# seang123/Masters-Thesis

Hardware: AMD Instinct MI355X
Metric: caption-tokens/sec training (20k-voxel enc, 512 LSTM, B=64) (higher is better)
Workload: dtype f32; 1 GPU; config 2: AttemptFour NIC.py dense 20000->512 encoder + BatchNorm + 512-unit LSTM, V=5001, T=15, B=64/GPU; global_batch=64, seq_len=15, parallelism=dp1, replay=launch plan

## Files before the change

### include/tnt_hip.h

```cpp
#ifndef TNT_HIP_H
#define TNT_HIP_H
#include <stdint.h>

#ifdef __cplusplus
extern "C" {
#endif

#define TNT_ACT_NONE 0
#define TNT_ACT_LEAKY 1
#define TNT_ACT_RELU 2
#define TNT_ACT_TANH 3

int32_t tnt_version(void);

int32_t tnt_gemm_f32(const float* A, const float* B, float* C, const float* bias, float* pre,
                     int32_t M, int32_t N, int32_t K, int32_t lda, int32_t ldb, int32_t ldc,
                     int32_t transA, int32_t transB, int32_t act, float slope,
                     int32_t accumulate, int32_t splitk, float* work, void* stream);
int32_t tnt_gemm_blas_f32(const float* A, const float* B, float* C, int32_t M, int32_t N, int32_t K,
                          int32_t lda, int32_t ldb, int32_t ldc, int32_t transA, int32_t transB,
                          int32_t accumulate, void* stream);

int32_t tnt_gemm_lt_f32(const float* A, const float* B, float* C, const float* bias, int32_t M, int32_t N, int32_t K,
                        int32_t lda, int32_t ldb, int32_t ldc, int32_t transA, int32_t transB, void* stream);
// ... 46 lines not shown
int32_t tnt_dense_dw_adam_fin_f32(const float* x, const float* dpre, float* theta, float* m, float* v, float l2,
                                  const float* partial, int32_t k0, int32_t k1, const float* sq_override,
                                  const float* lr_t_dev, float beta1, float beta2, float eps, float clipnorm,
                                  const uint32_t* guard, int32_t N, int32_t E, int32_t Bk, int32_t ldx, void* stream);
int32_t tnt_adam_fin_f32(float* theta, float* m, float* v, const float* grad, const int32_t* span_seg,
                         const int64_t* span_off, const int32_t* span_len, const float* sq_override, int32_t nspan, float eps,
                         float clipnorm, const tnt_finalize_desc* fin, const float* met, int32_t nmet, float* ring,
                         int32_t ring_rows, uint32_t* ring_t, void* stream);

int32_t tnt_gemm_f32_tile(const float* A, const float* B, float* C, const float* bias, float* pre,
                          int32_t M, int32_t N, int32_t K, int32_t lda, int32_t ldb, int32_t ldc,
                          int32_t transA, int32_t transB, int32_t act, float slope,
                          int32_t accumulate, int32_t splitk, float* work, int32_t bm, int32_t bn,
                          void* stream);

int32_t tnt_dropout_mask4_u8(uint8_t* out, int64_t n, int32_t nsites, float rate, uint64_t seed, uint32_t site0,
                             uint32_t step, const uint32_t* step_dev, void* stream);
int32_t tnt_dropout_f32(const float* x, float* y, int32_t rows, int32_t cols, int32_t ld,
                        int32_t tmajor_B, int32_t lwidth, int32_t lcol0, int32_t rows_per_site,
                        float rate, uint64_t seed, uint32_t site, uint32_t step,
                        const uint32_t* step_dev, void* stream);
int32_t tnt_dropout_metric_f32(const float* x, float* y, int32_t rows, int32_t cols, int32_t ld, int32_t tmajor_B,
                               int32_t lwidth, int32_t lcol0, int32_t rows_per_site, float rate, uint64_t seed,
                               uint32_t site, uint32_t step, const uint32_t* step_dev, const float* alpha,
                               float* partial, int32_t T, int32_t B, int32_t R, void* stream);
int32_t tnt_dropout2_f32(const float* x, float* y, int32_t rows, int32_t cols, int32_t ld, int32_t tmajor_B_a,
                         int32_t lwidth_a, int32_t lcol0_a, int32_t rows_per_site_a, float rate_a, uint32_t site_a,
                         int32_t tmajor_B_b, int32_t lwidth_b, int32_t lcol0_b, int32_t rows_per_site_b, float rate_b,
                         uint32_t site_b, uint64_t seed, uint32_t step, const uint32_t* step_dev, void* stream);

int32_t tnt_act_bwd_f32(const float* pre, const float* dy, float* dx, int64_t n, int32_t act,
                        float slope, void* stream);
int32_t tnt_bias_act_drop_bwd_f32(const float* dy, const float* pre, float* dx, float* dbias, int32_t rows, int32_t cols,
                                  int32_t ld, int32_t act, float slope, int32_t tmajor_B, int32_t lwidth, int32_t lcol0,
                                  float rate, uint64_t seed, uint32_t site, const uint32_t* step_dev, const float* x1,
                                  float* out1, int32_t rows1, int32_t C1, int32_t ld1, void* stream);

int32_t tnt_bn_nchunk(int32_t rows);
int32_t tnt_batchnorm_fwd_f32(const float* x, const float* gamma, const float* beta,
                              float* mov_mean, float* mov_var, float* y, float* xhat,
                              float* inv_std, int32_t rows, int32_t C, int32_t ldy,
                              int32_t training, float eps, float momentum, float* work,
                              void* stream);
int32_t tnt_batchnorm_fwd_drop_f32(const float* x, const float* gamma, const float* beta,
                                   float* mov_mean, float* mov_var, float* y, float* xhat,
                                   float* inv_std, int32_t rows, int32_t C, int32_t ldy,
                                   int32_t training, float eps, float momentum, float* work,
                                   float rate, uint64_t seed, uint32_t site, const uint32_t* step_dev,
                                   void* stream);
int32_t tnt_batchnorm_bwd_f32(const float* dy, const float* xhat, const float* gamma,
                              const float* inv_std, float* dx, float* dgamma, float* dbeta,
                              int32_t rows, int32_t C, int32_t lddy, int32_t training,
                              float* work, void* stream);
int32_t tnt_batchnorm_bwd_act_f32(const float* dy, const float* xhat, const float* gamma,
                              const float* inv_std, float* dx, float* dgamma, float* dbeta,
                              int32_t rows, int32_t C, int32_t lddy, int32_t training,
                              float* work, const float* act_pre, float slope, void* stream);

int32_t tnt_batchnorm_stats_f32(const float* x, int32_t rows, int32_t C, float* part, void* stream);
int32_t tnt_batchnorm_apply_stats_f32(const float* part_all, int32_t nrep, const float* x, const float* gamma,
                                      const float* beta, float* mov_mean, float* mov_var, float* y, float* xhat,
                                      float* inv_std, int32_t rows, int32_t C, int32_t ldy, float eps, float momentum,
                                      float* mean_work, void* stream);
int32_t tnt_batchnorm_dx_f32(const float* dy, int32_t lddy, const float* xhat, const float* gamma, const float* inv_std,
                             const float* dgamma_sum, const float* dbeta_sum, float* dx, int32_t rows, int32_t C,
                             int32_t n_total, void* stream);

int32_t tnt_locally_dense_fwd_split_f32(const float* x, int32_t ldx, const int32_t* idx, const int32_t* vgoff,
                                        const int32_t* vreg, const int32_t* rfirst, int32_t NV,
                                        const float* W, const float* bias, float* pre, float* y,
                                        float* partial, int32_t B, int32_t R, int32_t D, float slope,
                                        int32_t x_voxel_major, void* stream);
int32_t tnt_locally_dense_bwd_split_f32(const float* x, int32_t ldx, const int32_t* idx, const int32_t* vgoff,
                                        const int32_t* vreg, const int32_t* vfirst, int32_t NV,
                                        const float* dpre, float* dW, float* db, int32_t B, int32_t R,
                                        int32_t D, int32_t x_voxel_major, void* stream);

int32_t tnt_dense_fwd_stream_f32(const float* x, const float* w, float* part, int32_t B, int32_t E, int32_t K,
                                 int32_t ldx, int32_t ldw, int32_t nsplit, void* stream);

int32_t tnt_dense_fwd_stream_gram_f32(const float* x, const float* w, float* part, float* gx_part, float* w2_part,
                                      int32_t B, int32_t E, int32_t K, int32_t ldx, int32_t ldw, int32_t nsplit,
                                      void* stream);
int32_t tnt_dense_gram_norm_f32(const float* dpre, const float* pre, const float* bias, const float* gx_part,
                                int32_t nsplit, const float* w2_part, int32_t nw2, float l2, float* partial,
                                int32_t nslot, int32_t Bk, int32_t E, void* stream);
int32_t tnt_dense_gram_norm_spans_f32(const float* dpre, const float* pre, const float* bias, const float* gx_part,
                                      int32_t nsplit, const float* w2_part, int32_t nw2, float l2, float* partial,
                                      int32_t nslot, int32_t Bk, int32_t E, const float* theta, const float* grad,
                                      const int32_t* span_seg, const int64_t* span_off, const int32_t* span_len,
                                      const float* seg_l2, float* span_partial, int32_t nspan, void* stream);

int32_t tnt_dense_dw_skinny_f32(const float* x, const float* dpre, float* dw, int32_t N, int32_t E,
                                int32_t Bk, int32_t ldx, void* stream);

int32_t tnt_dense_dw_sqnorm_f32(const float* x, const float* dpre, const float* theta, float l2, float* partial,
                                int32_t nslot, int32_t N, int32_t E, int32_t Bk, int32_t ldx, void* stream);
int32_t tnt_dense_dw_adam_f32(const float* x, const float* dpre, float* theta, float* m, float* v, float l2,
                              const float* sq, const float* sq_override, const float* lr_t_dev, float beta1,
                              float beta2, float eps, float clipnorm, const uint32_t* guard, int32_t N, int32_t E,
                              int32_t Bk, int32_t ldx, void* stream);

int32_t tnt_enc_tail_fwd_f32(const float* y, const float* gamma, const float* beta, float* mov_mean,
                             float* mov_var, float* out, float* xhat, float* inv_std, int32_t rows,
                             int32_t C, int32_t ldo, int32_t training, float eps, float momentum,
                             float r_feat, float r_lstm, uint64_t seed, uint32_t site_feat,
                             uint32_t site_lstm, const uint32_t* step_dev, void* stream);
int32_t tnt_enc_tail_fwd_sk_f32(const float* part, int32_t nsplit, const float* bias, float* pre, float slope,
                                const float* gamma, const float* beta, float* mov_mean, float* mov_var, float* out,
                                float* xhat, float* inv_std, int32_t rows, int32_t C, int32_t ldo, int32_t training,
                                float eps, float momentum, float r_feat, float r_lstm, uint64_t seed,
                                uint32_t site_feat, uint32_t site_lstm, const uint32_t* step_dev, void* stream);
int32_t tnt_enc_tail_fwd_sk_emb_f32(const float* part, int32_t nsplit, const float* bias, float* pre, float slope,
                                    const float* gamma, const float* beta, float* mov_mean, float* mov_var, float* out,
                                    float* xhat, float* inv_std, int32_t rows, int32_t C, int32_t ldo, int32_t training,
                                    float eps, float momentum, float r_feat, float r_lstm, uint64_t seed,
                                    uint32_t site_feat, uint32_t site_lstm, const uint32_t* step_dev,
                                    const float* emb_table, const int32_t* emb_ids, float* emb_out, int32_t emb_B,
                                    int32_t emb_T, int32_t emb_V, float emb_rate, uint32_t emb_site, void* stream);
int32_t tnt_enc_tail_bwd_f32(const float* dout, const float* xhat, const float* gamma, const float* inv_std,
                             const float* pre, float* dpre, float* dgamma, float* dbeta, float* dbias,
                             int32_t rows, int32_t C, int32_t ldo, float r_feat, float r_lstm, float slope,
                             uint64_t seed, uint32_t site_feat, uint32_t site_lstm,
                             const uint32_t* step_dev, void* stream);
int32_t tnt_enc_tail_bwd_drop_f32(const float* dout, const float* xhat, const float* gamma, const float* inv_std,
                                  const float* pre, float* dpre, float* dgamma, float* dbeta, float* dbias, int32_t rows,
                                  int32_t C, int32_t ldo, float r_feat, float r_lstm, float slope, uint64_t seed,
                                  uint32_t site_feat, uint32_t site_lstm, const uint32_t* step_dev, float* drop_x,
                                  int32_t drop_rows, int32_t drop_cols, int32_t drop_ld, int32_t drop_tmajor_B,
                                  int32_t drop_lwidth, int32_t drop_lcol0, float drop_rate, uint32_t drop_site,
                                  void* stream);

int32_t tnt_layernorm_fwd_f32(const float* x, const float* gamma, const float* beta, float* y,
                              float* xhat, float* inv_std, int32_t rows, int32_t C,
                              int32_t ldy, float eps, void* stream);
int32_t tnt_layernorm_bwd_f32(const float* dy, const float* xhat, const float* gamma,
                              const float* inv_std, float* dx, float* dgamma, float* dbeta,
                              int32_t rows, int32_t C, int32_t lddy, float* work, void* stream);

int32_t tnt_colsum_f32(const float* x, float* out, int32_t rows, int32_t C, int32_t ld,
                       float* work, void* stream);
int32_t tnt_colsum4_f32(const float* x0, float* out0, int32_t rows0, int32_t C0, int32_t ld0, const float* x1, float* out1,
                        int32_t rows1, int32_t C1, int32_t ld1, const float* x2, float* out2, int32_t rows2, int32_t C2,
                        int32_t ld2, const float* x3, float* out3, int32_t rows3, int32_t C3, int32_t ld3, void* stream);
int32_t tnt_colsum2_f32(const float* x0, float* out0, int32_t rows0, int32_t C0, int32_t ld0, const float* x1,
                        float* out1, int32_t rows1, int32_t C1, int32_t ld1, void* stream);

int32_t tnt_embedding_fwd_f32(const float* table, const int32_t* ids, float* out, int32_t B,
                              int32_t T, int32_t E, int32_t ldo, int32_t V, void* stream);
int32_t tnt_embedding_fwd_drop_f32(const float* table, const int32_t* ids, float* out, float* out_drop,
                                   int32_t B, int32_t T, int32_t E, int32_t ldo, int32_t V, float rate,
                                   uint64_t seed, uint32_t site, uint32_t step, const uint32_t* step_dev,
                                   void* stream);
int32_t tnt_embedding_fwd_drop2_f32(const float* table, const int32_t* ids, float* out, float* out_drop,
                                    int32_t B, int32_t T, int32_t E, int32_t ldo, int32_t V, float rate,
                                    uint64_t seed, uint32_t site, uint32_t step, const uint32_t* step_dev,
                                    float rate2, uint32_t site2, int32_t lwidth2, int32_t lcol0_2, void* stream);
int32_t tnt_embedding_bwd_parts(int32_t B, int32_t T, int32_t E);
int32_t tnt_embedding_bwd_sparse_f32(const float* drows, const int32_t* ids, const int32_t* prev_ids, float* dtable,
                                     float* sq_part, int32_t B, int32_t T, int32_t E, int32_t ldd, int32_t V,
                                     float drop_rate, uint64_t drop_seed, uint32_t drop_site,
                                     const uint32_t* drop_step_dev, int32_t zero_id, void* stream);
int32_t tnt_embedding_bwd_f32(const float* drows, const int32_t* ids, float* dtable,
                              float* sq_norm, float* rowsq_work, int32_t B, int32_t T,
                              int32_t E, int32_t ldd, int32_t V, void* stream);

// ... 260 lines not shown
```

### masters-thesis_amd/_lib.py

```python
import ctypes as C
import os

import torch

_HERE = os.path.dirname(os.path.abspath(__file__))
LIB_PATH = os.environ.get("TNT_HIP_LIB") or os.path.join(_HERE, "csrc", "libtnt_hip.so")

P = C.c_void_p
I32, I64, U32, U64, F32 = C.c_int32, C.c_int64, C.c_uint32, C.c_uint64, C.c_float

SIGNATURES = {
    "tnt_version": [],
    "tnt_gemm_f32": [P, P, P, P, P, I32, I32, I32, I32, I32, I32, I32, I32, I32, F32, I32, I32, P, P],
    "tnt_gemm_fused_f32": [P, P, P, P, P, P, P, I32, I32, I32, I32, I32, I32, I32, I32, I32, P],
    "tnt_gemm_fused_cfg": [I32, I32, I32, I32, I32, I32],
    "tnt_gemm3_f32": [P, P, P, P, P, P, P, I32, I32, I32, I32, I32, I32, I32, I32, I32, I32, P, P, P, I32, P],
    "tnt_gemm3_plan": [I32, I32, I32, I32, I32, I32, I32, P, P],
    "tnt_gemm3_work_floats": [I32, I32, I32, I32, I32],
    "tnt_gemm3_sync_words": [I32, I32, I32, I32],
    "tnt_gemm3_work_arm": [P, I64, P],
    "tnt_gemm3_pair_supported": [I32, I32, I32, I32, I32, I32],
    "tnt_gemm3_pair_f32": [P, P, P],
    "tnt_span_sqnorm_lr_f32": [P, P, P, P, P, P, P, I32, P, P, P, F32, F32, P, P],
    "tnt_dense_gram_norm_spans_lr_f32": [P, P, P, P, I32, P, I32, F32, P, I32, I32, I32, P, P, P, P, P, P, P, I32, P, P, P, F32, F32, P, P],
    "tnt_dense_dw_adam_fin_f32": [P, P, P, P, P, F32, P, I32, I32, P, P, F32, F32, F32, F32, P, I32, I32, I32, I32, P],
    "tnt_adam_fin_f32": [P, P, P, P, P, P, P, P, I32, F32, F32, P, P, I32, P, I32, P, P],
    "tnt_dropout_mask4_u8": [P, I64, I32, F32, U64, U32, U32, P, P],
    "tnt_dropout_f32": [P, P, I32, I32, I32, I32, I32, I32, I32, F32, U64, U32, U32, P, P],
    "tnt_dropout_metric_f32": [P, P, I32, I32, I32, I32, I32, I32, I32, F32, U64, U32, U32, P, P, P, I32, I32, I32, P],
    "tnt_dropout2_f32": [P, P, I32, I32, I32, I32, I32, I32, I32, F32, U32, I32, I32, I32, I32, F32, U32, U64, U32, P, P],
    "tnt_act_bwd_f32": [P, P, P, I64, I32, F32, P],
    "tnt_bn_nchunk": [I32],
    "tnt_batchnorm_fwd_f32": [P, P, P, P, P, P, P, P, I32, I32, I32, I32, F32, F32, P, P],
    "tnt_batchnorm_bwd_f32": [P, P, P, P, P, P, P, I32, I32, I32, I32, P, P],
    "tnt_batchnorm_fwd_drop_f32": [P, P, P, P, P, P, P, P, I32, I32, I32, I32, F32, F32, P, F32, U64, U32, P, P],
    "tnt_batchnorm_bwd_act_f32": [P, P, P, P, P, P, P, I32, I32, I32, I32, P, P, F32, P],
    "tnt_batchnorm_stats_f32": [P, I32, I32, P, P],
    "tnt_batchnorm_apply_stats_f32": [P, I32, P, P, P, P, P, P, P, P, I32, I32, I32, F32, F32, P, P],
    "tnt_batchnorm_dx_f32": [P, I32, P, P, P, P, P, P, I32, I32, I32, P],
    "tnt_layernorm_fwd_f32": [P, P, P, P, P, P, I32, I32, I32, F32, P],
    "tnt_layernorm_bwd_f32": [P, P, P, P, P, P, P, I32, I32, I32, P, P],
    "tnt_colsum_f32": [P, P, I32, I32, I32, P, P],
    "tnt_bias_act_drop_bwd_f32": [P, P, P, P, I32, I32, I32, I32, F32, I32, I32, I32, F32, U64, U32, P, P, P, I32, I32, I32, P],
    "tnt_colsum2_f32": [P, P, I32, I32, I32, P, P, I32, I32, I32, P],
    "tnt_colsum4_f32": [P, P, I32, I32, I32, P, P, I32, I32, I32, P, P, I32, I32, I32, P, P, I32, I32, I32, P],
    "tnt_embedding_fwd_f32": [P, P, P, I32, I32, I32, I32, I32, P],
    "tnt_embedding_bwd_parts": [I32, I32, I32],
    "tnt_attention_front_bwd_parts": [I32, I32, I32],
    "tnt_attention_metric_parts": [I32, I32],
    "tnt_embedding_bwd_sparse_f32": [P, P, P, P, P, I32, I32, I32, I32, I32, F32, U64, U32, P, I32, P],
    "tnt_embedding_bwd_f32": [P, P, P, P, P, I32, I32, I32, I32, I32, P],
    "tnt_lstm_seq_supported": [I32, I32],
    "tnt_lstm_seq_fwd_f32": [P, P, P, P, P, P, I32, I32, P, P, I32, I32, I32, P, P, P, P],
    "tnt_lstm_seq_bwd_work_floats": [I32, I32],
    "tnt_lstm_seq_bwd_f32": [P, P, P, I32, I32, P, P, P, P, I64, I32, I32, I32, P, P, P, P],
    "tnt_lstm_step_fwd_f32": [P, P, P, P, P, P, I32, P, I32, I32, P, P, P, P, P, I32, I32, P, P],
    "tnt_ln_lstm_cell_fwd_f32": [P, P, P, P, P, P, P, P, P, P, P, I32, I32, F32, P],
    "tnt_ln_lstm_cell_bwd_f32": [P, P, P, P, P, P, P, P, P, P, P, P, P, I32, I32, P],
    "tnt_lstm_step_bwd_f32": [P, P, P, P, P, P, P, P, I32, I32, P, P, P, P, P, P, P, I32, I32, P, I32, P, P],
    "tnt_softmax_cce_f32": [P, P, P, P, P, P, I32, I32, I32, F32, I32, I32, P],
    "tnt_softmax_cce_live_f32": [P, P, P, P, P, P, I32, I32, I32, F32, P, P, P],
    "tnt_softmax_cce_smooth_f32": [P, P, P, P, P, P, I32, I32, I32, F32, F32, P],
    "tnt_softmax_cce_unlikely_f32": [P, P, P, P, P, P, I32, I32, I32, I32, F32, F32, P],
    "tnt_onehot_argmax_f32": [P, P, I32, I32, I32, P],
    "tnt_beam_topk_f32": [P, P, P, I32, I32, I32, I32, I32, P, P, P, P, P],
    "tnt_beam_step_f32": [P, I32, P, P, I32, I32, I32, I32, P, P, P, P, P, P, I32, I32, P, P, P],
    "tnt_beam_step_diverse_f32": [P, I32, P, P, I32, I32, I32, I32, P, P, P, P, P, P, I32, I32, P, P, I32, F32, P],
    "tnt_decode_constrain_f32": [P, I32, I32, I32, I32, P, P, I32, P, P, P, F32, I32, I32, I32, P, I32, P],
    "tnt_consensus_mix_f32": [P, I32, I32, I32, I32, P, I32, P, I32, P, P],
    "tnt_consensus_spread_i32": [P, P, P, I32, I32, P, P, P, P],
    "tnt_guidance_mix_f32": [P, I32, I32, I32, F32, F32, P, I32, P, P],
    "tnt_argmax_rows_f32": [P, P, I32, I32, I32, P],
    "tnt_greedy_feedback_f32": [P, I32, I32, P, I32, P, I32, I32, P, I32, I32, P, I32, P, I32, I32, F32, U64, U32, U32, P,
                                I32, I32, P],
    "tnt_scheduled_feedback_f32": [P, I32, I32, P, I32, P, I32, I32, P, I32, I32, P, I32, P, I32, I32, F32, U64, U32, U32, P,
                                   I32, I32, I32, I32, P, P, U32, U32, P],
    "tnt_scheduled_feedback2_f32": [P, I32, I32, P, I32, P, I32, I32, P, I32, I32, P, I32, P, I32, I32, F32, U64, U32, U32, P,
                                    I32, I32, I32, I32, P, P, U32, U32, F32, U32, I32, I32, P],
    "tnt_enc_tail_fwd_f32": [P, P, P, P, P, P, P, P, I32, I32, I32, I32, F32, F32, F32, F32, U64, U32, U32, P, P],
    "tnt_enc_tail_bwd_f32": [P, P, P, P, P, P, P, P, P, I32, I32, I32, F32, F32, F32, U64, U32, U32, P, P],
    "tnt_enc_tail_bwd_drop_f32": [P, P, P, P, P, P, P, P, P, I32, I32, I32, F32, F32, F32, U64, U32, U32, P, P, I32, I32, I32, I32,
                                  I32, I32, F32, U32, P],
    "tnt_embedding_fwd_drop_f32": [P, P, P, P, I32, I32, I32, I32, I32, F32, U64, U32, U32, P, P],
    "tnt_embedding_fwd_drop2_f32": [P, P, P, P, I32, I32, I32, I32, I32, F32, U64, U32, U32, P, F32, U32, I32, I32, P],
    "tnt_dense_dw_skinny_f32": [P, P, P, I32, I32, I32, I32, P],
    "tnt_dense_dw_sqnorm_f32": [P, P, P, F32, P, I32, I32, I32, I32, I32, P],
    "tnt_dense_dw_adam_f32": [P, P, P, P, P, F32, P, P, P, F32, F32, F32, F32, P, I32, I32, I32, I32, P],
    "tnt_dense_fwd_stream_gram_f32": [P, P, P, P, P, I32, I32, I32, I32, I32, I32, P],
    "tnt_dense_gram_norm_f32": [P, P, P, P, I32, P, I32, F32, P, I32, I32, I32, P],
    "tnt_dense_gram_norm_spans_f32": [P, P, P, P, I32, P, I32, F32, P, I32, I32, I32, P, P, P, P, P, P, P, I32, P],
    "tnt_dense_fwd_stream_f32": [P, P, P, I32, I32, I32, I32, I32, I32, P],
    "tnt_enc_tail_fwd_sk_f32": [P, I32, P, P, F32, P, P, P, P, P, P, P, I32, I32, I32, I32, F32, F32, F32, F32, U64, U32,
                                U32, P, P],
    "tnt_enc_tail_fwd_sk_emb_f32": [P, I32, P, P, F32, P, P, P, P, P, P, P, I32, I32, I32, I32, F32, F32, F32, F32, U64, U32,
                                    U32, P, P, P, P, I32, I32, I32, F32, U32, P],
    "tnt_gru_step_fwd_f32": [P, P, P, P, P, P, I32, I32, P],
    "tnt_gru_step_bwd_f32": [P, P, P, P, P, P, P, P, P, I32, I32, P],
    "tnt_lc_seq_fwd_f32": [P, P, P, P, P, P, P, P, P, P, P, I64, P, P, P, P, P, P, P, I32, I32, I32, I32, I32, I32, F32, F32, F32,
                           I32, U64, U32, U32, P, P, P, P, P],
    "tnt_lc_seq_fwd_work_floats": [I32],
    "tnt_lc_seq_bwd_f32": [P, P, P, P, P, P, P, I64, P, P, P, P, P, P, P, P, P, P, P, I32, I32, I32, I32, I32, I32, F32, F32, F32,
                           I32, U64, U32, U32, P, F32, P, P, P],
    "tnt_lc_seq_fwd_drop_f32": [P, P, P, P, P, P, P, P, P, P, P, I64, P, P, P, P, P, P, P, I32, I32, I32, I32, I32, I32, F32, F32,
                                F32, I32, U64, U32, U32, P, P, F32, U32, P, P, P, P],
    "tnt_lc_seq_bwd_drop_f32": [P, P, P, P, P, P, P, I64, P, P, P, P, P, P, P, P, P, P, P, I32, I32, I32, I32, I32, I32, F32, F32,
                                F32, I32, U64, U32, U32, P, F32, F32, U32, P, P, P],
    "tnt_lc_seq_bwd_work_floats": [I32, I32],
    "tnt_attention_front_bwd_f32": [P, P, P, P, P, P, P, P, I32, I32, I32, F32, P],
    "tnt_attention_front_bwd_drop_f32": [P, P, P, P, P, P, P, P, I32, I32, I32, F32, F32, U64, U32, P, P],
    "tnt_gemm_blas_f32": [P, P, P, I32, I32, I32, I32, I32, I32, I32, I32, I32, P],
    "tnt_gemm_lt_f32": [P, P, P, P, I32, I32, I32, I32, I32, I32, I32, I32, P],
    "tnt_locally_dense_fwd_split_f32": [P, I32, P, P, P, P, I32, P, P, P, P, P, I32, I32, I32, F32, I32, P],
    "tnt_locally_dense_bwd_split_f32": [P, I32, P, P, P, P, I32, P, P, P, I32, I32, I32, I32, P],
    "tnt_sum2_f32": [P, P, P, P, I32, F32, P],
    "tnt_stage_batch_f32": [P, P, P, P, P, P, P, P, P, P, I32, I32, I32, I32, I32, P, I32, P],
    "tnt_stage_batch_map_f32": [P, P, P, P, P, P, P, P, P, P, I32, I32, I32, I32, I32, P, I32, P, P, P, P, P, P, P],
    "tnt_stage_batch_h16": [P, P, P, P, P, P, P, P, P, P, I32, I32, I32, I32, I32, P, I32, P],
    "tnt_stage_batch_masks_f32": [P, P, P, P, P, P, P, P, P, P, I32, I32, I32, I32, I32, P, I32, P, I64, I32, F32, U64, U32, P, P],
    "tnt_scst_cce_f32": [P, I32, I32, P, I32, P, P, I32, P, P, P, I32, F32, P],
    "tnt_caption_score_f32": [P, I32, I32, P, I32, I32, I32, I32, P, P, P, P],
    "tnt_sample_rows_f32": [P, P, I32, I32, I32, F32, I32, U64, U32, U32, P, P],
    "tnt_sample_topkp_f32": [P, P, I32, I32, I32, F32, I32, F32, I32, U64, U32, U32, P, P],
    "tnt_sqdiff_mean_f32": [P, P, I64, F32, P],
    "tnt_sum_f32": [P, P, I32, F32, P],
    "tnt_l2_total_f32": [P, P, I32, P, P],
    "tnt_seg_sqnorm_f32": [P, P, P, P, P, P, P, P, P, P, P, I32, I32, P],
    "tnt_span_sqnorm_f32": [P, P, P, P, P, P, P, I32, P],
    "tnt_step_finalize_f32": [P, P, P, P, P, P, I32, P, P, P, P, I32, F32, P, P, I32, P, P, I32, P, P, I32, F32, P, P, P, P,
                              F32, F32, P, P],
    "tnt_adam_f32": [P, P, P, P, P, P, P, P, P, P, I32, F32, P, F32, F32, F32, F32, P, P],
    "tnt_adam_ring_f32": [P, P, P, P, P, P, P, P, P, P, I32, F32, P, F32, F32, F32, F32, P, P, I32, P, I32, P, P],
    "tnt_sgd_f32": [P, P, P, P, P, P, P, P, P, I32, F32, P, F32, F32, P, P],
    "tnt_agc_f32": [P, P, P, P, P, P, P, I32, P, P, I32, I32, I32, P, P, F32, F32, P],
    "tnt_colsq_f32": [P, P, I32, I32, I32, P],
    "tnt_step_tick": [P, P, P, P, F32, F32, P, P],
    "tnt_weight_average_f32": [P, P, I64, P, I32, P, I32, I64, I32, P, P],
    "tnt_swap_f32": [P, P, I64, P],
    "tnt_sam_f32": [P, P, P, P, P, P, P, P, P, I32, I32, F32, I32, P],
    "tnt_gemm_f32_tile": [P, P, P, P, P, I32, I32, I32, I32, I32, I32, I32, I32, I32, F32, I32, I32, P, I32, I32, P],
    "tnt_block_dense_dx_f32": [P, P, P, I32, I32, I32, I32, P],
    "tnt_locally_dense_fwd_f32": [P, I32, P, P, P, P, P, P, I32, I32, I32, F32, P],
    "tnt_locally_dense_bwd_f32": [P, I32, P, P, P, P, P, I32, I32, I32, P],
    "tnt_attention_step_fwd_f32": [P, P, P, P, P, P, P, P, P, P, P, P, I32, I32, I32, I32, I32, F32, F32, F32,
                                   I32, U64, U32, U32, U32, P, P, P],
    "tnt_attention_step_bwd_f32": [P, P, P, P, P, P, P, P, P, P, P, P, I32, I32, I32, I32, I32, F32, F32, F32,
                                   I32, U64, U32, U32, U32, P, P, P, P, I32, P, F32, I32, P],
    "tnt_attention_metric_f32": [P, P, P, I32, I32, I32, I64, P],
}

_lib = None


class KernelLibraryError(RuntimeError):
    pass


def load():
    global _lib
    if _lib is not None:
        return _lib
    if not os.path.exists(LIB_PATH):
        raise KernelLibraryError(
            f"HIP kernel library not built: {LIB_PATH} is missing. Run "
            "`python -c 'import __graft_entry__ as g; g.build()'` (or `make -C masters-thesis_amd/csrc`). "
            "There is no CPU fallback.")
    lib = C.CDLL(LIB_PATH)
    for name, argtypes in SIGNATURES.items():
        try:
            fn = getattr(lib, name)
        except AttributeError as e:
            raise KernelLibraryError(f"{LIB_PATH} does not export {name}") from e
# ... 10 lines not shown
```

### masters-thesis_amd/csrc/encoder.hip

```cpp
#include "tnt_common.h"
#include "tnt_fin.h"

namespace {

constexpr int KC = 128;
constexpr int XLD = KC + 2;
constexpr int MAXD = 64;
constexpr int WLD = MAXD + 16;

struct EncArgs {
  const float* x; int ldx; const int* idx; const int* goff; const float* W; const float* bias;
  float* pre; float* y; const float* dpre; float* dW; float* db;
  int B, R, D; float slope; int accumulate;
  const int* vgoff; const int* vreg; const int* vfirst; float* partial;
  int x_voxel_major;
};

__device__ __forceinline__ void gather_tile(const EncArgs& g, float* Xs, int* Is, int g0, int k0, int kc) {
  for (int k = threadIdx.x; k < kc; k += 256) Is[k] = g.idx[g0 + k0 + k];
  __syncthreads();
  if (g.x_voxel_major) {
    const int total4 = 16 * kc;
    for (int e0 = threadIdx.x; e0 < total4; e0 += 256 * 4) {
      float4 v[4];
#pragma unroll
      for (int u = 0; u < 4; ++u) {
        const int e = e0 + u * 256;
        const int k = e >> 4, r4 = (e & 15) * 4;
        v[u] = make_float4(0.f, 0.f, 0.f, 0.f);
        if (e < total4) {
          const float* src = g.x + (long)Is[k] * g.ldx + r4;
          if (r4 + 3 < g.B) v[u] = *reinterpret_cast<const float4*>(src);
          else { if (r4 < g.B) v[u].x = src[0]; if (r4 + 1 < g.B) v[u].y = src[1]; if (r4 + 2 < g.B) v[u].z = src[2]; }
        }
      }
#pragma unroll
      for (int u = 0; u < 4; ++u) {
        const int e = e0 + u * 256;
        if (e < total4) {
          const int k = e >> 4, r4 = (e & 15) * 4;
          Xs[(r4 + 0) * XLD + k] = v[u].x; Xs[(r4 + 1) * XLD + k] = v[u].y;
          Xs[(r4 + 2) * XLD + k] = v[u].z; Xs[(r4 + 3) * XLD + k] = v[u].w;
        }
      }
    }
    return;
  }
  const int total = 64 * kc;
  for (int e0 = threadIdx.x; e0 < total; e0 += 256 * 8) {
    float v[8];
#pragma unroll
    for (int u = 0; u < 8; ++u) {
      const int e = e0 + u * 256;
      const int row = e / kc, k = e % kc;
      v[u] = (e < total && row < g.B) ? g.x[(long)row * g.ldx + Is[k]] : 0.f;
    }
#pragma unroll
    for (int u = 0; u < 8; ++u) {
      const int e = e0 + u * 256;
      if (e < total) Xs[(e / kc) * XLD + e % kc] = v[u];
    }
  }
}

__global__ __launch_bounds__(256) void locally_dense_fwd_kernel(EncArgs g) {
  __shared__ float Xs[64 * XLD];
  __shared__ float Ws[KC * WLD];
  __shared__ int Is[KC];
  const int vr = blockIdx.x, tid = threadIdx.x, lane = tid & 63, w = tid >> 6;
  const int kq = lane >> 4, lr = lane & 15;
  const int r = g.vreg ? g.vreg[vr] : vr;
  const int g0 = g.vreg ? g.vgoff[vr] : g.goff[r], nr = (g.vreg ? g.vgoff[vr + 1] : g.goff[r + 1]) - g0;
  const int DT = g.D / 16;
  floatx4 acc[MAXD / 16];
#pragma unroll
  for (int c = 0; c < MAXD / 16; ++c) acc[c] = (floatx4){0.f, 0.f, 0.f, 0.f};
  for (int k0 = 0; k0 < nr; k0 += KC) {
    const int kc = min(KC, nr - k0);
    const int kc4 = (kc + 3) & ~3;
    __syncthreads();
    gather_tile(g, Xs, Is, g0, k0, kc);
    for (int e = tid; e < 64 * (kc4 - kc); e += 256) Xs[(e / (kc4 - kc)) * XLD + kc + e % (kc4 - kc)] = 0.f;
    for (int e = tid; e < kc4 * g.D; e += 256) {
      const int k = e / g.D, d = e % g.D;
// ... 296 lines not shown
    }
    lr_t = a.lr_t_dev[0];
  }
  __syncthreads();
  for (; s < nstrip; s += gridDim.x, cur ^= 1) {
    float av[DW_KS];
#pragma unroll
    for (int ks = 0; ks < DW_KS; ++ks) av[ks] = As[cur][(4 * ks + lk) * DW_LDA + lc];
    sstore(cur ^ 1);
    if (EPI == 0 && sprev >= 0) store_strip(outp, sprev);
    gload(s + 2 * gridDim.x);
    if (EPI >= 1) {
#pragma unroll
      for (int r = 0; r < 4; ++r) {
        th[r] = thn[r];
        if (EPI == 2) { mm[r] = mmn[r]; vv[r] = vvn[r]; }
      }
      tload(s + gridDim.x, thn, mmn, vvn);
    }
    floatx4 acc[DW_MAXT];
#pragma unroll
    for (int j = 0; j < DW_MAXT; ++j) acc[j] = (floatx4){0.f, 0.f, 0.f, 0.f};
#pragma unroll
    for (int ks = 0; ks < DW_KS; ++ks)
#pragma unroll
      for (int j = 0; j < DW_MAXT; ++j) acc[j] = __builtin_amdgcn_mfma_f32_16x16x4f32(av[ks], bq[ks][j], acc[j], 0, 0, 0);
    if (EPI == 0) {
#pragma unroll
      for (int j = 0; j < DW_MAXT; ++j) outp[j] = acc[j];
    } else {
#pragma unroll
      for (int r = 0; r < 4; ++r) {
        if (s * DW_MS + lk * 4 + r >= a.N) continue;
        const float g4[4] = {acc[0][r], acc[TPW > 1 ? 1 : 0][r], acc[TPW > 2 ? 2 : 0][r], acc[TPW > 3 ? 3 : 0][r]};
        float* wp = &th[r].x;
        if (EPI == 1) {
#pragma unroll
          for (int j = 0; j < 4; ++j) {
            const float a0 = g4[j] + a.lam2 * wp[j];
            q += a0 * a0; wq += wp[j] * wp[j];
          }
        } else {
          float* mp = &mm[r].x; float* vp = &vv[r].x;
          const float ob1 = 1.f - a.b1, ob2 = 1.f - a.b2;
#pragma unroll
          for (int j = 0; j < 4; ++j) {
            const float g = (g4[j] + a.lam2 * wp[j]) * cs;
            mp[j] = mp[j] + (g - mp[j]) * ob1;
            vp[j] = vp[j] + (g * g - vp[j]) * ob2;
            wp[j] = wp[j] - lr_t * mp[j] / (sqrtf(vp[j]) + a.eps);
          }
          const long o = (long)s * DW_MS * a.E + (long)r * a.E + eoff;
          *reinterpret_cast<float4*>(a.theta + o) = th[r];
          tnt_st4<NTM>(a.m + o, mm[r]);
          tnt_st4<NTM>(a.v + o, vv[r]);
        }
      }
    }
    sprev = s;
    asm volatile("s_waitcnt lgkmcnt(0)\n\ts_barrier" ::: "memory");
  }
  if (EPI == 0 && sprev >= 0) store_strip(outp, sprev);
  if (EPI == 1) {
    __shared__ float rq[8], rw[8];
    q = tnt_wave_sum(q); wq = tnt_wave_sum(wq);
    if (lane == 0) { rq[w] = q; rw[w] = wq; }
    __syncthreads();
    if (tid == 0) {
      float sq_ = 0.f, sw_ = 0.f;
#pragma unroll
      for (int k = 0; k < 8; ++k) { sq_ += rq[k]; sw_ += rw[k]; }
      const int slot = blockIdx.y * gridDim.x + blockIdx.x, nwg = gridDim.x * gridDim.y;
      a.partial[2 * slot] = sq_; a.partial[2 * slot + 1] = sw_;
      for (int k = slot + nwg; k < a.nslot; k += nwg) { a.partial[2 * k] = 0.f; a.partial[2 * k + 1] = 0.f; }
    }
  }
}
}

namespace {
constexpr int DF_CW = 32;

struct DfArgs { const float* x; const float* w; float* part; int B, E, K, ldx, ldw, nsplit; float* gx_part; float* w2_part; };

template <int NW, int DEPTH, bool GRAM>
__global__ __launch_bounds__(64 * NW) void dense_fwd_stream_kernel(DfArgs a) {
  __shared__ float red[NW][64][DF_CW + 4];
  const int tid = threadIdx.x, lane = tid & 63, kq = lane >> 4, ln = lane & 15;
  const int w = __builtin_amdgcn_readfirstlane(tid >> 6);
  const int nct = a.E / DF_CW;
  int ct, split;
  if (a.nsplit % 8 == 0) {
    const int xcd = blockIdx.x & 7, slot = blockIdx.x >> 3;
    ct = slot % nct; split = xcd * (a.nsplit / 8) + slot / nct;
  } else {
    ct = blockIdx.x % nct; split = blockIdx.x / nct;
  }
  const int c0 = ct * DF_CW, rb = blockIdx.y * 64;
  const int nslot = a.nsplit * NW, q = split * NW + w;
  const int Tfull = a.K / 16;
  const int nt = q < Tfull ? (Tfull - q + nslot - 1) / nslot : 0;
  unsigned aoff[4], boff[4];
#pragma unroll
  for (int rt = 0; rt < 4; ++rt) aoff[rt] = ((unsigned)min(rb + rt * 16 + ln, a.B - 1) * a.ldx + kq * 4) * 4u;
#pragma unroll
  for (int j = 0; j < 4; ++j) boff[j] = ((unsigned)(kq * 4 + j) * a.ldw + c0 + 2 * ln) * 4u;
  floatx4 acc[4][2];
#pragma unroll
  for (int rt = 0; rt < 4; ++rt)
#pragma unroll
    for (int c = 0; c < 2; ++c) acc[rt][c] = (floatx4){0.f, 0.f, 0.f, 0.f};
  float4 av[DEPTH][4];
  float2 bv[DEPTH][4];
  floatx4 accg = {0.f, 0.f, 0.f, 0.f};
  float w2 = 0.f;
  const int g_rt = (ct >> 2) & 3, g_rtp = ct & 3;
  float ga[4], gb[4];
#pragma unroll
  for (int t = 0; t < 4; ++t) { ga[t] = g_rt == t ? 1.f : 0.f; gb[t] = g_rtp == t ? 1.f : 0.f; }
  auto load = [&](int s, int tile) {
    const int tc = max(min(tile, Tfull - 1), 0);
    const char* xb = reinterpret_cast<const char*>(a.x) + (size_t)tc * 64;
    const char* wb = reinterpret_cast<const char*>(a.w) + (size_t)tc * 64 * a.ldw;
#pragma unroll
    for (int rt = 0; rt < 4; ++rt) av[s][rt] = *reinterpret_cast<const float4*>(xb + aoff[rt]);
#pragma unroll
    for (int j = 0; j < 4; ++j) bv[s][j] = *reinterpret_cast<const float2*>(wb + boff[j]);
  };
  auto mac = [&](int s) {
#pragma unroll
    for (int j = 0; j < 4; ++j) {
#pragma unroll
      for (int rt = 0; rt < 4; ++rt) {
        const float4 v = av[s][rt];
        const float x = j == 0 ? v.x : j == 1 ? v.y : j == 2 ? v.z : v.w;
        acc[rt][0] = __builtin_amdgcn_mfma_f32_16x16x4f32(x, bv[s][j].x, acc[rt][0], 0, 0, 0);
        acc[rt][1] = __builtin_amdgcn_mfma_f32_16x16x4f32(x, bv[s][j].y, acc[rt][1], 0, 0, 0);
      }
    }
  };
  auto gram = [&](int s) {
#pragma unroll
    for (int j = 0; j < 4; ++j) {
      auto el = [&](int t) { const float4 v = av[s][t]; return j == 0 ? v.x : j == 1 ? v.y : j == 2 ? v.z : v.w; };
      const float xa = el(0) * ga[0] + el(1) * ga[1] + el(2) * ga[2] + el(3) * ga[3];
      const float xb = el(0) * gb[0] + el(1) * gb[1] + el(2) * gb[2] + el(3) * gb[3];
      accg = __builtin_amdgcn_mfma_f32_16x16x4f32(xa, xb, accg, 0, 0, 0);
      w2 += bv[s][j].x * bv[s][j].x + bv[s][j].y * bv[s][j].y;
    }
  };
#pragma unroll
  for (int s = 0; s < DEPTH - 1; ++s) load(s, q + s * nslot);
  int i = 0;
  for (; i + DEPTH <= nt; i += DEPTH) {
#pragma unroll
    for (int s = 0; s < DEPTH; ++s) {
      if (GRAM && i + s > 0) {
        gram((s + DEPTH - 1) % DEPTH);
        __builtin_amdgcn_sched_barrier(0);
      }
      load((s + DEPTH - 1) % DEPTH, q + (i + s + DEPTH - 1) * nslot);
      mac(s);
#pragma unroll
      for (int g = 0; g < 8; ++g) {
        __builtin_amdgcn_sched_group_barrier(0x008, 4, 0);
        __builtin_amdgcn_sched_group_barrier(0x020, 1, 0);
      }
      __builtin_amdgcn_sched_barrier(0);
    }
  }
  if (GRAM && i > 0) gram(DEPTH - 1);
#pragma unroll
  for (int s = 0; s < DEPTH - 1; ++s)
    if (i + s < nt) {
      mac(s);
      if (GRAM) gram(s);
    }
  if ((a.K & 15) && q == Tfull % nslot) {
    const int k0 = Tfull * 16 + kq * 4, ka = min(k0, a.K - 4);
    const float keep = k0 < a.K ? 1.f : 0.f;
#pragma unroll
    for (int rt = 0; rt < 4; ++rt) {
      const float4 v = *reinterpret_cast<const float4*>(a.x + (long)min(rb + rt * 16 + ln, a.B - 1) * a.ldx + ka);
      av[0][rt] = make_float4(v.x * keep, v.y * keep, v.z * keep, v.w * keep);
    }
#pragma unroll
    for (int j = 0; j < 4; ++j) bv[0][j] = *reinterpret_cast<const float2*>(a.w + (long)(ka + j) * a.ldw + c0 + 2 * ln);
    mac(0);
  }
#pragma unroll
  for (int rt = 0; rt < 4; ++rt)
#pragma unroll
    for (int r = 0; r < 4; ++r)
      *reinterpret_cast<float2*>(&red[w][rt * 16 + kq * 4 + r][2 * ln]) = make_float2(acc[rt][0][r], acc[rt][1][r]);
  __syncthreads();
  for (int e = tid; e < 64 * (DF_CW / 4); e += 64 * NW) {
    const int row = e / (DF_CW / 4), c4 = (e % (DF_CW / 4)) * 4;
    if (rb + row >= a.B) continue;
    float4 t = *reinterpret_cast<const float4*>(&red[0][row][c4]);
#pragma unroll
    for (int k = 1; k < NW; ++k) {
      const float4 u = *reinterpret_cast<const float4*>(&red[k][row][c4]);
      t.x += u.x; t.y += u.y; t.z += u.z; t.w += u.w;
    }
    *reinterpret_cast<float4*>(a.part + ((long)split * a.B + rb + row) * a.E + c0 + c4) = t;
  }
  if (GRAM && blockIdx.y == 0) {
    __syncthreads();
    float* rg = &red[0][0][0];
#pragma unroll
    for (int r = 0; r < 4; ++r) rg[(w * 16 + kq * 4 + r) * 17 + ln] = accg[r];
    w2 = tnt_wave_sum(w2);
    if (lane == 0) rg[NW * 16 * 17 + w] = w2;
    __syncthreads();
    if (tid < 256 && ct < 16) {
      const int row = tid >> 4, col = tid & 15;
      float t = 0.f;
#pragma unroll
      for (int k = 0; k < NW; ++k) t += rg[(k * 16 + row) * 17 + col];
      a.gx_part[((long)split * 64 + g_rt * 16 + row) * 64 + g_rtp * 16 + col] = t;
    }
    if (tid == 0) {
      float t = 0.f;
#pragma unroll
      for (int k = 0; k < NW; ++k) t += rg[NW * 16 * 17 + k];
      a.w2_part[split * nct + ct] = t;
    }
  }
}
}

static int32_t dense_fwd_stream_launch(const float* x, const float* w, float* part, float* gx_part, float* w2_part,
                                       int32_t B, int32_t E, int32_t K, int32_t ldx, int32_t ldw, int32_t nsplit,
                                       void* stream) {
  if (B <= 0 || K < 4 || K % 4 != 0 || ldx < K || ldx % 4 != 0) return TNT_BADARG(6);
  if (E <= 0 || E % DF_CW != 0 || ldw < E || ldw % 2 != 0 || nsplit <= 0 || nsplit > 64) return TNT_BADARG(5);
  if (!tnt_aligned16(x) || !tnt_aligned16(w) || !tnt_aligned16(part)) return TNT_BADARG(1);
  if ((long)B * ldx * 4 >= (1L << 32) || 16L * ldw * 4 >= (1L << 32)) return TNT_BADARG(4);
  DfArgs a{x, w, part, B, E, K, ldx, ldw, nsplit, gx_part, w2_part};
  const dim3 g((E / DF_CW) * nsplit, (B + 63) / 64);
  if (gx_part) hipLaunchKernelGGL((dense_fwd_stream_kernel<4, 4, true>), g, dim3(256), 0, tnt_stream(stream), a);
  else hipLaunchKernelGGL((dense_fwd_stream_kernel<4, 4, false>), g, dim3(256), 0, tnt_stream(stream), a);
  TNT_LAUNCH_CHECK();
  return 0;
}

extern "C" int32_t tnt_dense_fwd_stream_f32(const float* x, const float* w, float* part, int32_t B, int32_t E,
                                            int32_t K, int32_t ldx, int32_t ldw, int32_t nsplit, void* stream) {
  return dense_fwd_stream_launch(x, w, part, nullptr, nullptr, B, E, K, ldx, ldw, nsplit, stream);
}

extern "C" int32_t tnt_dense_fwd_stream_gram_f32(const float* x, const float* w, float* part, float* gx_part,
                                                 float* w2_part, int32_t B, int32_t E, int32_t K, int32_t ldx,
                                                 int32_t ldw, int32_t nsplit, void* stream) {
  if (gx_part == nullptr || w2_part == nullptr || E / DF_CW < 16 || K % 16 != 0 || B > 64) return TNT_BADARG(4);
  return dense_fwd_stream_launch(x, w, part, gx_part, w2_part, B, E, K, ldx, ldw, nsplit, stream);
}

namespace {
constexpr int GN_Q = 4;
struct GnSpans {
  const float* theta; const float* grad; const int32_t* span_seg; const int64_t* span_off; const int32_t* span_len;
  const float* seg_l2; float* partial; int nspan;
  const int64_t* adam_t; const float* lr; float* lr_t; float b1, b2;
  const float* ovr;
};

__global__ __launch_bounds__(256) void dense_gram_norm_kernel(const float* dpre, const float* pre, const float* bias,
                                                              const float* gx_part, int nsplit, const float* w2_part,
                                                              int nw2, float l2, float* partial, int nslot, int Bk, int E,
                                                              GnSpans sp) {
  __shared__ double sd[256];
  const int tid = threadIdx.x;
  if ((int)blockIdx.x > GN_Q * Bk) {
    __shared__ float s0[4], s1[4];
    const int s = blockIdx.x - (GN_Q * Bk + 1);
    if (s >= sp.nspan) return;
    const SpanTab st{sp.span_seg, sp.span_off, sp.span_len, nullptr, sp.seg_l2};
    tnt_span_norm(sp.theta, sp.grad, st, s, sp.partial, sp.ovr, s0, s1);
    return;
  }
  if ((int)blockIdx.x == GN_Q * Bk) {
    if (sp.lr_t != nullptr && tid == 255) sp.lr_t[0] = tnt_adam_lr_t(sp.adam_t, sp.lr, sp.b1, sp.b2);
    for (int k = tid; k < nslot - GN_Q * Bk; k += 256) {
      const float w = k < nw2 ? w2_part[k] : 0.f;
      partial[2 * (GN_Q * Bk + k)] = 4.f * l2 * l2 * w;
      partial[2 * (GN_Q * Bk + k) + 1] = w;
    }
    return;
  }
  const int b = blockIdx.x / GN_Q, qd = blockIdx.x % GN_Q;
  const int bp = qd * 16 + (tid >> 4), part = tid & 15;
  double acc = 0.0;
  if (bp < Bk) {
    const int n4 = E / 64;
    const float4* db = reinterpret_cast<const float4*>(dpre + (long)b * E) + part * n4;
    const float4* dp = reinterpret_cast<const float4*>(dpre + (long)bp * E) + part * n4;
#pragma unroll 8
    for (int e = 0; e < n4; ++e) {
      const float4 u = db[e], v = dp[e];
      acc += (double)u.x * (double)v.x + (double)u.y * (double)v.y + (double)u.z * (double)v.z + (double)u.w * (double)v.w;
    }
  }
#pragma unroll
  for (int o = 8; o > 0; o >>= 1) acc += __shfl_xor(acc, o, 16);
  double s = 0.0;
  if (part == 0 && bp < Bk) {
    double gx = 0.0;
#pragma unroll 8
    for (int sp = 0; sp < nsplit; ++sp) gx += (double)gx_part[((long)sp * 64 + b) * 64 + bp];
    s = gx * acc;
  }
  if (qd == 0) {
    double s2 = 0.0;
#pragma unroll 4
    for (int e = tid; e < E; e += 256) s2 += (double)dpre[(long)b * E + e] * ((double)pre[(long)b * E + e] - (double)bias[e]);
    s += 4.0 * (double)l2 * s2;
  }
  sd[tid] = s;
  __syncthreads();
  for (int k = 128; k > 0; k >>= 1) {
    if (tid < k) sd[tid] += sd[tid + k];
    __syncthreads();
  }
  if (tid == 0) { partial[2 * blockIdx.x] = (float)sd[0]; partial[2 * blockIdx.x + 1] = 0.f; }
}
}

static int32_t gram_norm_launch(const float* dpre, const float* pre, const float* bias, const float* gx_part, int32_t nsplit,
                                const float* w2_part, int32_t nw2, float l2, float* partial, int32_t nslot, int32_t Bk,
                                int32_t E, const GnSpans& sp, void* stream) {
  if (Bk <= 0 || Bk > 64 || E <= 0 || E % 64 != 0 || nsplit <= 0 || nw2 <= 0 || nslot < GN_Q * Bk + nw2) return TNT_BADARG(9);
// ... 151 lines not shown
```

### masters-thesis_amd/csrc/rowops.hip

```cpp
#include "tnt_common.h"
#include <hip/hip_fp16.h>
#include "tnt_rng.h"

namespace {

constexpr int MAX_CHUNKS = 128;
inline int chunk_count(int rows) { int n = (rows + 63) / 64; return n > MAX_CHUNKS ? MAX_CHUNKS : (n < 1 ? 1 : n); }
inline int chunk_rows(int rows) { const int n = chunk_count(rows); return (rows + n - 1) / n; }

struct DropArgs {
  const float* x; float* y; int rows, cols, ld, tB, lwidth, lcol0, rows_per_site;
  float rate, scale; uint64_t seed; uint32_t site, step; const uint32_t* step_dev;
};

__device__ __forceinline__ void drop_row(const DropArgs& a, int r, int T, long& lrow, uint32_t& site) {
  site = a.site;
  if (a.rows_per_site > 0) { site += (uint32_t)(r / a.rows_per_site); r = r % a.rows_per_site; }
  lrow = a.tB > 0 ? (long)(r % a.tB) * T + r / a.tB : r;
}

__global__ __launch_bounds__(256) void dropout_kernel(DropArgs a) {
  const uint32_t step = a.step + (a.step_dev ? a.step_dev[0] : 0u);
  const long total = (long)a.rows * a.cols;
  const int T = a.tB > 0 ? a.rows / a.tB : 0;
  for (long e = (long)blockIdx.x * 256 + threadIdx.x; e < total; e += (long)gridDim.x * 256) {
    const int r = (int)(e / a.cols), c = (int)(e % a.cols);
    long lrow; uint32_t site;
    drop_row(a, r, T, lrow, site);
    const uint64_t le = (uint64_t)lrow * (uint64_t)a.lwidth + (uint64_t)(a.lcol0 + c);
    const bool k = tnt_keep(le, a.rate, a.seed, site, step);
    const long o = (long)r * a.ld + c;
    a.y[o] = k ? a.x[o] * a.scale : 0.f;
  }
}

__global__ __launch_bounds__(256) void dropout4_kernel(DropArgs a) {
  const uint32_t step = a.step + (a.step_dev ? a.step_dev[0] : 0u);
  const int c4n = a.cols >> 2;
  const long total = (long)a.rows * c4n;
  const int T = a.tB > 0 ? a.rows / a.tB : 0;
  for (long e = (long)blockIdx.x * 256 + threadIdx.x; e < total; e += (long)gridDim.x * 256) {
    const int r = (int)(e / c4n), c = (int)(e % c4n) * 4;
    long lrow; uint32_t site;
    drop_row(a, r, T, lrow, site);
    const uint64_t le = (uint64_t)lrow * (uint64_t)a.lwidth + (uint64_t)(a.lcol0 + c);
    bool k[4];
    tnt_keep4(le, a.rate, a.seed, site, step, k);
    const long o = (long)r * a.ld + c;
    const float4 v = *reinterpret_cast<const float4*>(a.x + o);
    float4 w;
    w.x = k[0] ? v.x * a.scale : 0.f; w.y = k[1] ? v.y * a.scale : 0.f;
    w.z = k[2] ? v.z * a.scale : 0.f; w.w = k[3] ? v.w * a.scale : 0.f;
    *reinterpret_cast<float4*>(a.y + o) = w;
  }
}

__global__ __launch_bounds__(256) void dropout4x2_kernel(DropArgs a, DropArgs b) {
  const uint32_t step = a.step + (a.step_dev ? a.step_dev[0] : 0u);
  const int c4n = a.cols >> 2;
  const long total = (long)a.rows * c4n;
  const int Ta = a.tB > 0 ? a.rows / a.tB : 0, Tb = b.tB > 0 ? b.rows / b.tB : 0;
  for (long e = (long)blockIdx.x * 256 + threadIdx.x; e < total; e += (long)gridDim.x * 256) {
    const int r = (int)(e / c4n), c = (int)(e % c4n) * 4;
    long lrow; uint32_t site;
    bool ka[4], kb[4];
    drop_row(a, r, Ta, lrow, site);
    tnt_keep4((uint64_t)lrow * (uint64_t)a.lwidth + (uint64_t)(a.lcol0 + c), a.rate, a.seed, site, step, ka);
    drop_row(b, r, Tb, lrow, site);
    tnt_keep4((uint64_t)lrow * (uint64_t)b.lwidth + (uint64_t)(b.lcol0 + c), b.rate, b.seed, site, step, kb);
    const long o = (long)r * a.ld + c;
    const float4 v = *reinterpret_cast<const float4*>(a.x + o);
    float4 w;
    w.x = ka[0] ? v.x * a.scale : 0.f; w.y = ka[1] ? v.y * a.scale : 0.f;
    w.z = ka[2] ? v.z * a.scale : 0.f; w.w = ka[3] ? v.w * a.scale : 0.f;
    w.x = kb[0] ? w.x * b.scale : 0.f; w.y = kb[1] ? w.y * b.scale : 0.f;
    w.z = kb[2] ? w.z * b.scale : 0.f; w.w = kb[3] ? w.w * b.scale : 0.f;
    *reinterpret_cast<float4*>(a.y + o) = w;
  }
}

__global__ __launch_bounds__(256) void dropout_mask4_kernel(uint8_t* out, long n4, long total, float rate, uint64_t seed,
                                                            uint32_t site0, uint32_t step, const uint32_t* step_dev) {
  const uint32_t st = step + (step_dev ? step_dev[0] : 0u);
  for (long g = (long)blockIdx.x * 256 + threadIdx.x; g < total; g += (long)gridDim.x * 256) {
    const long k = g / n4, gi = g - k * n4;
// ... 189 lines not shown
                                                    const float* inv_std, const float* dgamma, const float* dbeta,
                                                    float* dx, int rows, int C, int training, int n_total,
                                                    const float* act_pre, float slope) {
  const long total = (long)rows * C;
  const float n = (float)n_total;
  for (long e = (long)blockIdx.x * 256 + threadIdx.x; e < total; e += (long)gridDim.x * 256) {
    const int r = (int)(e / C), c = (int)(e % C);
    const float g = dy[(long)r * lddy + c];
    const float k = gamma[c] * inv_std[c];
    float d = training ? k / n * (n * g - dbeta[c] - xhat[e] * dgamma[c]) : k * g;
    if (act_pre) d = tnt_act_grad(act_pre[e], d, 1, slope);
    dx[e] = d;
  }
}

__global__ __launch_bounds__(256) void ln_fwd_kernel(const float* x, const float* gamma, const float* beta, float* y,
                                                     float* xhat, float* inv_std, int rows, int C, int ldy, float eps) {
  const int row = blockIdx.x * 4 + (threadIdx.x >> 6), lane = threadIdx.x & 63;
  if (row >= rows) return;
  const float* xr = x + (long)row * C;
  float s = 0.f;
  for (int c = lane; c < C; c += 64) s += xr[c];
  const float mean = tnt_wave_sum(s) / C;
  float q = 0.f;
  for (int c = lane; c < C; c += 64) { const float d = xr[c] - mean; q += d * d; }
  const float inv = 1.f / sqrtf(tnt_wave_sum(q) / C + eps);
  if (lane == 0) inv_std[row] = inv;
  for (int c = lane; c < C; c += 64) {
    const float xh = (xr[c] - mean) * inv;
    xhat[(long)row * C + c] = xh;
    y[(long)row * ldy + c] = xh * gamma[c] + beta[c];
  }
}

__global__ __launch_bounds__(256) void ln_dx_kernel(const float* dy, int lddy, const float* xhat, const float* gamma,
                                                    const float* inv_std, float* dx, int rows, int C) {
  const int row = blockIdx.x * 4 + (threadIdx.x >> 6), lane = threadIdx.x & 63;
  if (row >= rows) return;
  float s0 = 0.f, s1 = 0.f;
  for (int c = lane; c < C; c += 64) {
    const float d = dy[(long)row * lddy + c] * gamma[c];
    s0 += d;
    s1 += d * xhat[(long)row * C + c];
  }
  s0 = tnt_wave_sum(s0); s1 = tnt_wave_sum(s1);
  const float k = inv_std[row] / C;
  for (int c = lane; c < C; c += 64) {
    const float d = dy[(long)row * lddy + c] * gamma[c];
    dx[(long)row * C + c] = k * (C * d - s0 - xhat[(long)row * C + c] * s1);
  }
}

__global__ __launch_bounds__(1024) void sum_kernel(const float* x, float* out, int n, float scale) {
  __shared__ float sw[16];
  float s = 0.f;
  for (int i = threadIdx.x; i < n; i += 1024) s += x[i];
  s = tnt_wave_sum(s);
  if ((threadIdx.x & 63) == 0) sw[threadIdx.x >> 6] = s;
  __syncthreads();
  if (threadIdx.x == 0) {
    float t = 0.f;
    for (int w = 0; w < 16; ++w) t += sw[w];
    out[0] = t * scale;
  }
}

__global__ __launch_bounds__(1024) void sum2_kernel(const float* x0, float* out0, const float* x1, float* out1, int n,
                                                    float scale) {
  __shared__ float sw[16];
  const float* x = blockIdx.x == 0 ? x0 : x1;
  float* out = blockIdx.x == 0 ? out0 : out1;
  float s = 0.f;
  for (int i = threadIdx.x; i < n; i += 1024) s += x[i];
  s = tnt_wave_sum(s);
  if ((threadIdx.x & 63) == 0) sw[threadIdx.x >> 6] = s;
  __syncthreads();
  if (threadIdx.x == 0) {
    float t = 0.f;
    for (int w = 0; w < 16; ++w) t += sw[w];
    out[0] = t * scale;
  }
}

template <typename XT>
struct StageArgs {
  const XT* x; float* xd; const int* cap; int* capd; const int* tgt; int* tgtd;
  const float* a0; float* h0; const float* c0; float* c0d;
  int B, T, N, ldx, U;
  float* xT; int ldt; int ncopy;
  uint8_t* mk_out; long mk_n4, mk_total; float mk_rate; uint64_t mk_seed; uint32_t mk_site0; const uint32_t* mk_step_dev;
  int nstage;
  int* map_pos; float* map_w; int* map_tgt; int* map_live; float* map_loss; float* map_corr;
};
constexpr int STAGE_MAP_LDS = 1024;
template <typename SA>
__device__ __forceinline__ void stage_rowmap_lds(const SA& a, int* lds) {
  int* s_cap = lds; int* s_tgt = lds + STAGE_MAP_LDS; int* s_pos = lds + 2 * STAGE_MAP_LDS; int* s_cnt = lds + 3 * STAGE_MAP_LDS;
  const int B = a.B, T = a.T, n = B * T, tid = threadIdx.x;
  for (int i = tid; i < n; i += 256) { s_cap[i] = a.cap[i]; s_tgt[i] = a.tgt[i]; }
  __syncthreads();
  for (int b = tid; b < B; b += 256) {
    int rep_y = 0;
    for (int t = 0; t < T; ++t) {
      const int id = s_cap[b * T + t], y = s_tgt[b * T + t];
      const bool merged = t > 0 && id == 0 && y == rep_y;
      s_pos[t * B + b] = merged ? -1 : 1;
      if (!merged) rep_y = y;
    }
  }
  __syncthreads();
  const int per = (n + 255) / 256, lo = min(tid * per, n), hi = min(lo + per, n);
  int c = 0;
  for (int i = lo; i < hi; ++i) c += s_pos[i] > 0 ? 1 : 0;
  s_cnt[tid] = c;
  __syncthreads();
  if (tid == 0) {
    int run = 0;
    for (int k = 0; k < 256; ++k) { const int v = s_cnt[k]; s_cnt[k] = run; run += v; }
    s_cnt[256] = run;
    a.map_live[0] = run;
  }
  __syncthreads();
  int idx = s_cnt[tid];
  const int live = s_cnt[256];
  for (int i = lo; i < hi; ++i)
    if (s_pos[i] > 0) s_pos[i] = idx++;
  __syncthreads();
  for (int b = tid; b < B; b += 256) {
    int rep = -1, cnt = 0;
    for (int t = 0; t < T; ++t) {
      const int p = s_pos[t * B + b];
      if (p >= 0) {
        if (rep >= 0) a.map_w[rep] = (float)cnt;
        rep = p; cnt = 1;
        a.map_tgt[p] = s_tgt[b * T + t];
      } else {
        ++cnt;
      }
    }
    if (rep >= 0) a.map_w[rep] = (float)cnt;
  }
  for (int i = tid; i < n; i += 256) a.map_pos[i] = s_pos[i];
  for (int i = live + tid; i < n; i += 256) {
    a.map_w[i] = 0.f; a.map_tgt[i] = 0;
    if (a.map_loss) a.map_loss[i] = 0.f;
    if (a.map_corr) a.map_corr[i] = 0.f;
  }
}
template <typename SA>
__device__ __forceinline__ void stage_rowmap(const SA& a, int* s_cnt) {
  const int B = a.B, T = a.T, n = B * T, tid = threadIdx.x;
  for (int b = tid; b < B; b += 256) {
    int rep_y = 0;
    for (int t = 0; t < T; ++t) {
      const int id = a.cap[b * T + t], y = a.tgt[b * T + t];
      const bool merged = t > 0 && id == 0 && y == rep_y;
      a.map_pos[t * B + b] = merged ? -1 : 1;
      if (!merged) rep_y = y;
    }
  }
  __syncthreads();
  const int per = (n + 255) / 256, lo = min(tid * per, n), hi = min(lo + per, n);
  int c = 0;
  for (int i = lo; i < hi; ++i) c += a.map_pos[i] > 0 ? 1 : 0;
  s_cnt[tid] = c;
  __syncthreads();
  if (tid == 0) {
    int run = 0;
    for (int k = 0; k < 256; ++k) { const int v = s_cnt[k]; s_cnt[k] = run; run += v; }
    s_cnt[256] = run;
    a.map_live[0] = run;
  }
  __syncthreads();
  int idx = s_cnt[tid];
  const int live = s_cnt[256];
  for (int i = lo; i < hi; ++i)
    if (a.map_pos[i] > 0) a.map_pos[i] = idx++;
  __syncthreads();
  for (int b = tid; b < B; b += 256) {
    int rep = -1, cnt = 0;
    for (int t = 0; t < T; ++t) {
      const int p = a.map_pos[t * B + b];
      if (p >= 0) {
        if (rep >= 0) a.map_w[rep] = (float)cnt;
        rep = p; cnt = 1;
        a.map_tgt[p] = a.tgt[b * T + t];
      } else {
        ++cnt;
      }
    }
    if (rep >= 0) a.map_w[rep] = (float)cnt;
  }
  for (int i = live + tid; i < n; i += 256) {
    a.map_w[i] = 0.f; a.map_tgt[i] = 0;
    if (a.map_loss) a.map_loss[i] = 0.f;
    if (a.map_corr) a.map_corr[i] = 0.f;
  }
}
__device__ __forceinline__ float stage_ld(const float* p) { return *p; }
__device__ __forceinline__ float stage_ld(const __half* p) { return __half2float(*p); }
__device__ __forceinline__ float4 stage_ld4(const float* p) { return *reinterpret_cast<const float4*>(p); }
__device__ __forceinline__ float4 stage_ld4(const __half* p) {
  const uint2 u = *reinterpret_cast<const uint2*>(p);
  const __half2 lo = *reinterpret_cast<const __half2*>(&u.x), hi = *reinterpret_cast<const __half2*>(&u.y);
  const float2 a = __half22float2(lo), b = __half22float2(hi);
  return make_float4(a.x, a.y, b.x, b.y);
}
template <typename XT, bool MAP>
__global__ __launch_bounds__(256) void stage_batch_kernel(StageArgs<XT> a) {
  __shared__ float tile[64][65];
  static_assert(sizeof(tile) >= (3 * STAGE_MAP_LDS + 257) * sizeof(int), "the row map's LDS arrays live in the tile");
  if (MAP && blockIdx.x == gridDim.x - 1) {
    int* lds = reinterpret_cast<int*>(&tile[0][0]);
    if (a.B * a.T <= STAGE_MAP_LDS) stage_rowmap_lds(a, lds);
    else stage_rowmap(a, lds);
    return;
  }
  if ((int)blockIdx.x >= a.nstage) {
    const uint32_t st = a.mk_step_dev ? a.mk_step_dev[0] : 0u;
    const long nb = gridDim.x - a.nstage - (MAP ? 1 : 0);
    for (long g = (long)(blockIdx.x - a.nstage) * 256 + threadIdx.x; g < a.mk_total; g += nb * 256) {
      const long k = g / a.mk_n4, gi = g - k * a.mk_n4;
      bool kp[4];
      tnt_keep4((uint64_t)gi * 4u, a.mk_rate, a.mk_seed, a.mk_site0 + (uint32_t)k, st, kp);
      a.mk_out[g] = (uint8_t)((kp[0] ? 1 : 0) | (kp[1] ? 2 : 0) | (kp[2] ? 4 : 0) | (kp[3] ? 8 : 0));
    }
    return;
  }
  if ((int)blockIdx.x >= a.ncopy) {
    const int ntc = (a.N + 63) / 64, ntr = (a.B + 63) / 64;
    for (int t = blockIdx.x - a.ncopy; t < ntc * ntr; t += a.nstage - a.ncopy) {
      const int c0 = (t % ntc) * 64, r0 = (t / ntc) * 64;
      __syncthreads();
      for (int e = threadIdx.x; e < 64 * 64; e += 256) {
        const int r = e >> 6, c = e & 63;
        tile[r][c] = (r0 + r < a.B && c0 + c < a.N) ? stage_ld(a.x + (long)(r0 + r) * a.N + c0 + c) : 0.f;
      }
      __syncthreads();
      for (int e = threadIdx.x; e < 64 * 64; e += 256) {
        const int c = e >> 6, r = e & 63;
        if (c0 + c < a.N && r0 + r < a.ldt) a.xT[(long)(c0 + c) * a.ldt + r0 + r] = tile[r][c];
      }
    }
    return;
  }
  const long gid = (long)blockIdx.x * 256 + threadIdx.x, gsz = (long)a.ncopy * 256;
  if (a.N % 4 == 0 && a.ldx % 4 == 0) {
    const int n4 = a.N / 4;
    for (long e = gid; e < (long)a.B * n4; e += gsz) {
      const int r = (int)(e / n4), c = (int)(e % n4) * 4;
      *reinterpret_cast<float4*>(a.xd + (long)r * a.ldx + c) = stage_ld4(a.x + (long)r * a.N + c);
    }
  } else {
    for (long e = gid; e < (long)a.B * a.N; e += gsz) {
      const int r = (int)(e / a.N), c = (int)(e % a.N);
      a.xd[(long)r * a.ldx + c] = stage_ld(a.x + e);
    }
  }
  const int bt = a.B * a.T, bu = a.B * a.U;
  for (long e = gid; e < bt; e += gsz) {
    a.capd[e] = a.cap[e];
    if (a.tgt) { const int b = (int)(e / a.T), t = (int)(e % a.T); a.tgtd[t * a.B + b] = a.tgt[e]; }
  }
  for (long e = gid; e < bu; e += gsz) { a.h0[e] = a.a0[e]; a.c0d[e] = a.c0[e]; }
}

inline int ew_blocks(long total) {
  long b = (total + 255) / 256;
  return (int)(b > 2048 ? 2048 : (b < 1 ? 1 : b));
}

}

extern "C" int32_t tnt_bn_nchunk(int32_t rows) { return chunk_count(rows); }

extern "C" int32_t tnt_dropout_f32(const float* x, float* y, int32_t rows, int32_t cols, int32_t ld, int32_t tmajor_B,
                                   int32_t lwidth, int32_t lcol0, int32_t rows_per_site, float rate, uint64_t seed,
                                   uint32_t site, uint32_t step, const uint32_t* step_dev, void* stream) {
  if (rows <= 0 || cols <= 0) return 0;
  const int rsite = rows_per_site > 0 ? rows_per_site : rows;
  if (tmajor_B > 0 && rsite % tmajor_B != 0) return TNT_BADARG(6);
  if (rows_per_site > 0 && tmajor_B > 0) return TNT_BADARG(9);
  DropArgs a;
  a.x = x; a.y = y; a.rows = rows; a.cols = cols; a.ld = ld; a.tB = tmajor_B; a.lwidth = lwidth; a.lcol0 = lcol0;
  a.rows_per_site = rows_per_site; a.rate = rate; a.scale = 1.0f / (1.0f - rate); a.seed = seed; a.site = site;
  a.step = step; a.step_dev = step_dev;
  const bool vec = ((cols | ld | lwidth | lcol0) & 3) == 0 && tnt_aligned16(x) && tnt_aligned16(y);
  if (vec)
    hipLaunchKernelGGL(dropout4_kernel, dim3(ew_blocks((long)rows * (cols / 4))), dim3(256), 0, tnt_stream(stream), a);
  else
    hipLaunchKernelGGL(dropout_kernel, dim3(ew_blocks((long)rows * cols)), dim3(256), 0, tnt_stream(stream), a);
  TNT_LAUNCH_CHECK();
  return 0;
}

__global__ __launch_bounds__(256) void dropout4_metric_kernel(DropArgs a, int nd, const float* alpha, float* partial, int B,
                                                              int R, int nc) {
  if ((int)blockIdx.x >= nd) {
    __shared__ float sb[4][64];
    const int k = blockIdx.x - nd, t = k / nc, c = k % nc, lane = threadIdx.x & 63, w = threadIdx.x >> 6;
    const int r = c * 64 + lane;
    float s = 0.f;
    if (r < R) {
#pragma unroll 8
      for (int b = w; b < B; b += 4) s += alpha[((long)t * B + b) * R + r];
    }
    sb[w][lane] = s;
    __syncthreads();
    if (w != 0) return;
    float acc = 0.f;
    if (r < R) {
      const float tot = ((sb[0][lane] + sb[1][lane]) + sb[2][lane]) + sb[3][lane];
      acc = (1.f - tot) * (1.f - tot);
    }
    acc = tnt_wave_sum(acc);
    if (lane == 0) partial[k] = acc;
    return;
  }
  const uint32_t step = a.step + (a.step_dev ? a.step_dev[0] : 0u);
  const int c4n = a.cols >> 2;
  const long total = (long)a.rows * c4n;
  const int T = a.tB > 0 ? a.rows / a.tB : 0;
  for (long e = (long)blockIdx.x * 256 + threadIdx.x; e < total; e += (long)nd * 256) {
    const int r = (int)(e / c4n), c = (int)(e % c4n) * 4;
    long lrow; uint32_t site;
    drop_row(a, r, T, lrow, site);
    const uint64_t le = (uint64_t)lrow * (uint64_t)a.lwidth + (uint64_t)(a.lcol0 + c);
    bool k[4];
    tnt_keep4(le, a.rate, a.seed, site, step, k);
    const long o = (long)r * a.ld + c;
    const float4 v = *reinterpret_cast<const float4*>(a.x + o);
    float4 w;
    w.x = k[0] ? v.x * a.scale : 0.f; w.y = k[1] ? v.y * a.scale : 0.f;
    w.z = k[2] ? v.z * a.scale : 0.f; w.w = k[3] ? v.w * a.scale : 0.f;
    *reinterpret_cast<float4*>(a.y + o) = w;
  }
}

extern "C" int32_t tnt_dropout_metric_f32(const float* x, float* y, int32_t rows, int32_t cols, int32_t ld, int32_t tmajor_B,
                                          int32_t lwidth, int32_t lcol0, int32_t rows_per_site, float rate, uint64_t seed,
                                          uint32_t site, uint32_t step, const uint32_t* step_dev, const float* alpha,
                                          float* partial, int32_t T, int32_t B, int32_t R, void* stream) {
  if (rows <= 0 || cols <= 0 || T <= 0 || B <= 0 || R <= 0 || alpha == nullptr || partial == nullptr) return TNT_BADARG(3);
  const int rsite = rows_per_site > 0 ? rows_per_site : rows;
  if (tmajor_B > 0 && rsite % tmajor_B != 0) return TNT_BADARG(6);
  if (rows_per_site > 0 && tmajor_B > 0) return TNT_BADARG(9);
  if (((cols | ld | lwidth | lcol0) & 3) != 0 || !tnt_aligned16(x) || !tnt_aligned16(y)) return TNT_BADARG(1);
// ... 731 lines not shown
  hipLaunchKernelGGL(sum2_kernel, dim3(2), dim3(1024), 0, tnt_stream(stream), x0, out0, x1, out1, n, scale);
  TNT_LAUNCH_CHECK();
  return 0;
}

namespace {
template <typename XT>
int32_t stage_batch_launch(const XT* x, float* x_dst, const int32_t* cap, int32_t* cap_dst, const int32_t* tgt,
                           int32_t* tgt_tmajor, const float* a0, float* h0, const float* c0, float* c0_dst, int32_t B,
                           int32_t T, int32_t N, int32_t ldx, int32_t U, float* xT_dst, int32_t ldt, void* stream,
                           uint8_t* keep_out = nullptr, int64_t keep_n = 0, int32_t keep_sites = 0, float keep_rate = 0.f,
                           uint64_t keep_seed = 0, uint32_t keep_site0 = 0, const uint32_t* keep_step_dev = nullptr,
                           int32_t* map_pos = nullptr, float* map_w = nullptr, int32_t* map_tgt = nullptr,
                           int32_t* map_live = nullptr, float* map_loss = nullptr, float* map_corr = nullptr) {
  if (B <= 0 || T <= 0 || N <= 0 || ldx < N || U <= 0) return TNT_BADARG(11);
  if (map_pos != nullptr && (map_w == nullptr || map_tgt == nullptr || map_live == nullptr || tgt == nullptr)) return TNT_BADARG(19);
  if (keep_out != nullptr && (keep_n <= 0 || keep_n % 4 != 0 || keep_sites <= 0)) return TNT_BADARG(19);
  if (xT_dst && ldt < B) return TNT_BADARG(16);
  const bool vec = (N % 4 == 0) && (ldx % 4 == 0);
  const bool src_ok = sizeof(XT) == 4 ? tnt_aligned16(x) : ((reinterpret_cast<uintptr_t>(x) & 7u) == 0);
  if (vec && (!src_ok || !tnt_aligned16(x_dst))) return TNT_BADARG(1);
  StageArgs<XT> a{};
  a.x = x; a.xd = x_dst; a.cap = cap; a.capd = cap_dst; a.tgt = tgt; a.tgtd = tgt_tmajor; a.a0 = a0; a.h0 = h0; a.c0 = c0;
  a.c0d = c0_dst; a.B = B; a.T = T; a.N = N; a.ldx = ldx; a.U = U; a.xT = xT_dst; a.ldt = ldt;
  a.ncopy = ew_blocks((long)B * N / (vec ? 4 : 1));
  int nt = 0;
  if (xT_dst) { nt = ((N + 63) / 64) * ((B + 63) / 64); if (nt > 1024) nt = 1024; }
  a.nstage = a.ncopy + nt;
  long nmask = 0;
  if (keep_out) {
    a.mk_out = keep_out; a.mk_n4 = keep_n / 4; a.mk_total = a.mk_n4 * keep_sites; a.mk_rate = keep_rate; a.mk_seed = keep_seed;
    a.mk_site0 = keep_site0; a.mk_step_dev = keep_step_dev;
    nmask = (a.mk_total + 255) / 256;
    if (nmask > 8192) nmask = 8192;
  }
  a.map_pos = map_pos; a.map_w = map_w; a.map_tgt = map_tgt; a.map_live = map_live; a.map_loss = map_loss; a.map_corr = map_corr;
  if (map_pos != nullptr)
    hipLaunchKernelGGL((stage_batch_kernel<XT, true>), dim3(a.nstage + (int)nmask + 1), dim3(256), 0, tnt_stream(stream), a);
  else
    hipLaunchKernelGGL((stage_batch_kernel<XT, false>), dim3(a.nstage + (int)nmask), dim3(256), 0, tnt_stream(stream), a);
  TNT_LAUNCH_CHECK();
  return 0;
}
}

extern "C" int32_t tnt_stage_batch_f32(const float* x, float* x_dst, const int32_t* cap, int32_t* cap_dst,
                                       const int32_t* tgt, int32_t* tgt_tmajor, const float* a0, float* h0,
                                       const float* c0, float* c0_dst, int32_t B, int32_t T, int32_t N, int32_t ldx,
                                       int32_t U, float* xT_dst, int32_t ldt, void* stream) {
  return stage_batch_launch<float>(x, x_dst, cap, cap_dst, tgt, tgt_tmajor, a0, h0, c0, c0_dst, B, T, N, ldx, U, xT_dst,
                                   ldt, stream);
}

extern "C" int32_t tnt_stage_batch_map_f32(const float* x, float* x_dst, const int32_t* cap, int32_t* cap_dst,
                                           const int32_t* tgt, int32_t* tgt_tmajor, const float* a0, float* h0,
                                           const float* c0, float* c0_dst, int32_t B, int32_t T, int32_t N, int32_t ldx,
                                           int32_t U, float* xT_dst, int32_t ldt, int32_t* pos, float* row_weight,
                                           int32_t* tgt_compact, int32_t* live, float* loss_row, float* corr_row,
                                           void* stream) {
  if (pos == nullptr) return TNT_BADARG(17);
  return stage_batch_launch<float>(x, x_dst, cap, cap_dst, tgt, tgt_tmajor, a0, h0, c0, c0_dst, B, T, N, ldx, U, xT_dst,
                                   ldt, stream, nullptr, 0, 0, 0.f, 0, 0, nullptr, pos, row_weight, tgt_compact, live,
                                   loss_row, corr_row);
}

extern "C" int32_t tnt_stage_batch_masks_f32(const float* x, float* x_dst, const int32_t* cap, int32_t* cap_dst,
                                             const int32_t* tgt, int32_t* tgt_tmajor, const float* a0, float* h0,
                                             const float* c0, float* c0_dst, int32_t B, int32_t T, int32_t N, int32_t ldx,
                                             int32_t U, float* xT_dst, int32_t ldt, uint8_t* keep_out, int64_t keep_n,
                                             int32_t keep_sites, float keep_rate, uint64_t keep_seed, uint32_t keep_site0,
                                             const uint32_t* keep_step_dev, void* stream) {
  return stage_batch_launch<float>(x, x_dst, cap, cap_dst, tgt, tgt_tmajor, a0, h0, c0, c0_dst, B, T, N, ldx, U, xT_dst,
                                   ldt, stream, keep_out, keep_n, keep_sites, keep_rate, keep_seed, keep_site0, keep_step_dev);
}

extern "C" int32_t tnt_stage_batch_h16(const uint16_t* x_half, float* x_dst, const int32_t* cap, int32_t* cap_dst,
                                       const int32_t* tgt, int32_t* tgt_tmajor, const float* a0, float* h0,
                                       const float* c0, float* c0_dst, int32_t B, int32_t T, int32_t N, int32_t ldx,
                                       int32_t U, float* xT_dst, int32_t ldt, void* stream) {
  return stage_batch_launch<__half>(reinterpret_cast<const __half*>(x_half), x_dst, cap, cap_dst, tgt, tgt_tmajor, a0,
                                    h0, c0, c0_dst, B, T, N, ldx, U, xT_dst, ldt, stream);
}

extern "C" int32_t tnt_version(void) { return 119; }
```

### masters-thesis_amd/model_base.py

```python
import time
from collections import OrderedDict
from contextlib import contextmanager, nullcontext

import numpy as np
import torch

from . import ops
from .optimizers import Adam, loss_label_smoothing, loss_unlikelihood, optimizer_average

S_IN, S_FEAT, S_TEXT, S_OUT = 1, 2, 3, 5
S_ATTN, S_LSTM_IN, S_LSTM_OUT = 16, 48, 80
S_SAMPLE = 112
S_SS_COIN, S_SS_DRAW = 176, 208
SS_MAX_POSITIONS = 32
S_SCST_LAST = 240
BN_EPS, BN_MOMENTUM = 1e-3, 0.99


SCORE_LOGITS_BYTES = 256 << 20


class ScheduledSampling:

    KINDS = ("linear", "inverse_sigmoid")
# ... 1151 lines not shown
    @contextmanager
    def averaged_weights(self):
        self._average_buf("averaged_weights")
        if self._swapped:
            raise RuntimeError("the averaged weights are already swapped in")
        self.swap_weights()
        try:
            yield self
        finally:
            self.swap_weights()

    def assign_average_vars(self):
        avg = self._average_buf("assign_average_vars")
        if self._swapped:
            raise RuntimeError("the averaged weights are swapped in: swap back before assign_average_vars")
        self.arena.theta.copy_(avg)

    def get_layer(self, name):
        if name not in self.layers_spec:
            raise ValueError(f"No such layer: {name}")
        return _LayerView(self, name, self.layers_spec[name])

    def save_weights(self, path, averaged=False):
        path = str(path)
        get = self.get_weight
        if averaged:
            self._average_buf("save_weights(averaged=True)")
            get = lambda n: self.get_optimizer_slot(n, "average") if n in self.arena.entries else self.get_weight(n)
        if path.endswith((".h5", ".hdf5")):
            from . import h5lite
            layers = OrderedDict((layer, [(f"{layer}/{w}:0", get(f"{layer}/{w}")) for w in ws])
                                 for layer, ws in self.layers_spec.items())
            h5lite.write_keras_weights(path, layers)
            return
        arrs = {n.replace("/", "__"): get(n) for n in self.keras_shapes}
        with open(path, "wb") as f:
            np.savez(f, **arrs)

    def load_weights(self, path, by_name=True, skip_mismatch=False, name_map=None):
        path = str(path)
        name_map = name_map or {}
        items = []
        if path.endswith((".h5", ".hdf5")):
            from . import h5lite
            _, layers = h5lite.read_keras_weights(path)
            for ln, ws in layers.items():
                tgt = name_map.get(ln, ln)
                for wn, arr in ws:
                    w = wn.split("/")[-1].split(":")[0]
                    items.append((f"{tgt}/{w}", arr))
        else:
            with np.load(path, allow_pickle=False) as z:
                items = [(name_map.get(k.replace("__", "/"), k.replace("__", "/")), z[k]) for k in z.files]
        for n, arr in items:
            if n not in self.keras_shapes:
                continue
            if tuple(arr.shape) != tuple(self.keras_shapes[n]):
                if skip_mismatch:
                    continue
                raise ValueError(f"shape mismatch for {n}: {arr.shape} vs {self.keras_shapes[n]}")
            self.set_weight(n, arr)

    def count_params(self):
        return int(sum(np.prod(s) for s in self.keras_shapes.values()))

    def summary(self, print_fn=print):
        print_fn(f'Model: "{type(self).__name__}"')
        for layer, ws in self.layers_spec.items():
            n = sum(int(np.prod(self.keras_shapes[f"{layer}/{w}"])) for w in ws)
            print_fn(f"  {layer:36s} {n:>12,d}")
        print_fn(f"Total params: {self.count_params():,d}")

    def _to_dev(self, a, dtype):
        if isinstance(a, torch.Tensor):
            return a.to(device=self.device, dtype=dtype, non_blocking=True)
        return torch.as_tensor(np.asarray(a), dtype=dtype).to(self.device, non_blocking=True)

    def _stage_mask_job(self):
        return None

    def _head_map_bufs(self, B, T):
        return None

    def _stage_batch(self, inputs, target, n_cols, masks=False, head_map=False):
        x, cap, a0, c0 = inputs[:4]
        if target is not None and self.unlikelihood > 0 and np.shape(cap)[-1] > self.UNLIKELIHOOD_MAX_T:
            raise ValueError(f"unlikelihood training holds a caption's prefix in one wave: at most {self.UNLIKELIHOOD_MAX_T} "
                             f"loss positions per caption, got {np.shape(cap)[-1]}")
        ts = [x, cap, a0, c0] + ([target] if target is not None else [])
        dev = self.device
        same = lambda t: t.device.type == dev.type and (t.device.index or 0) == (dev.index or 0)
        ok = all(isinstance(t, torch.Tensor) and same(t) and t.is_contiguous() for t in ts)
        ok = ok and x.dtype in (torch.float32, torch.float16) and a0.dtype == c0.dtype == torch.float32
        ok = ok and cap.dtype == torch.int32
        ok = ok and x.dim() == 2 and cap.dim() == 2 and x.shape == (cap.shape[0], n_cols)
        ok = ok and (target is None or (target.dtype == torch.int32 and target.shape == cap.shape))
        self._head_map_fresh = False
        if not ok:
            B, T = self._stage_inputs(inputs)
            if target is not None:
                self._stage_target(target, B, T)
            mk = self._stage_mask_job() if masks else None
            if mk is not None:
                self.be.dropout_mask4(mk[0], mk[1], mk[2], mk[3], mk[4], mk[5], 0, mk[6])
            return B, T
        B, T = cap.shape
        self._build(B, T)
        assert a0.shape == c0.shape == (B, self.U), f"state shape {tuple(a0.shape)} != {(B, self.U)}"
        xT = getattr(self, "xT", None)
        kw = {}
        mk = self._stage_mask_job() if masks else None
        if mk is not None:
            kw["masks"] = mk
        hm = self._head_map_bufs(B, T) if (head_map and target is not None and mk is None and xT is None
                                           and x.dtype == torch.float32) else None
        if hm is not None:
            self.be.stage_batch_map(x, self.x, cap, self.cap, target, self.tgt, a0, self.Hs[0], c0, self.Cs[0], B, T, n_cols,
                                    self.ldx, self.U, *hm)
            self._head_map_fresh = True
        elif xT is not None:
            self.be.stage_batch(x, self.x, cap, self.cap, target, self.tgt, a0, self.Hs[0], c0, self.Cs[0], B, T, n_cols,
                                self.ldx, self.U, xT, xT.shape[1], **kw)
        else:
            self.be.stage_batch(x, self.x, cap, self.cap, target, self.tgt, a0, self.Hs[0], c0, self.Cs[0], B, T, n_cols,
                                self.ldx, self.U, **kw)
        return B, T

    def _stage_target(self, target, B, T):
        if isinstance(target, np.ndarray) and target.ndim == 2 or (isinstance(target, torch.Tensor) and target.dim() == 2):
            t = self._to_dev(target, torch.int32)
            self.tgt.view(T, B).copy_(t.t())
        else:
            oh = self._to_dev(target, torch.float32).contiguous()
            assert oh.shape == (B, T, self.V), f"target shape {tuple(oh.shape)}"
            self.be.onehot_argmax(oh, self.tgt, B, T, self.V)

    def _guard_word(self):
        sync = self.__dict__.get("seq_sync")
        return sync[1024:1025] if (sync is not None and self.__dict__.get("_seq_lstm")) else None

    def _guard_out(self):
        return self.met[self.GUARD:self.GUARD + 1]

    def _seq_chain(self, bwd=False):
        if not self._seq_lstm or (bwd and self.seq_xch is None):
            return None
        return (self.seq_sync, self._guard_out()) + ((self.seq_xch,) if bwd else ())

    def _run_step(self, run, key, fn):
        graphs = self.use_graph and self.device.type == "cuda"
        st = self._graphs.get(key) if graphs else None
        executed = (not graphs) or st is None or (isinstance(st, str) and st == "warm")
        self._ring_hit = False
        run(key, fn)
        keys = self.__dict__.setdefault("_ring_keys", set())
        if executed or self._ring_hit:
            (keys.add if self._ring_hit else keys.discard)(key)
        return key in keys

    def _met_snapshot(self, ring=False):
        if ring:
            t = self._ring_host
            self._ring_host = t + 1
            row = self.met_ring[t % self.METRIC_RING]
            self._last_ring = (row, t & 0xFFFFFF)
            return row
        self._last_ring = None
        return self.met.clone()

    def _ring_args(self):
        if not getattr(self, "metric_ring", True) or self.__dict__.get("met") is None or self.met.numel() > 62:
            return {}
        if self.__dict__.get("met_ring") is None or self.met_ring.shape[1] != self.met.numel() + 1:
            if self.device.type == "cuda" and torch.cuda.is_current_stream_capturing():
                return {}
            self.met_ring = self._f(self.METRIC_RING, self.met.numel() + 1)
            self.ring_t = torch.zeros(1, dtype=torch.int32, device=self.device)
            self._ring_host = 0
            self._graphs = {}
        self._ring_hit = True
        return dict(met=self.met, ring=self.met_ring, ring_t=self.ring_t)

    def _metrics_from(self, m, **slots):
        out = Metrics((k, m[i] if isinstance(i, int) else i) for k, i in slots.items())
        out._ring = self.__dict__.get("_last_ring")
        return out.guarded(self, m[self.GUARD]) if self.__dict__.get("_seq_lstm") else out

    def _on_guard_trip(self, code):
        self.disable_seq_lstm()
        what = {1: "a barrier timed out", 2: "a launch did not place 32 workgroups on every XCD"}.get(code, "unknown")
        raise DeviceGuardError(
            f"persistent LSTM kernel: device guard tripped (code {code}: {what}).  The results of that step are invalid; "
            "its optimizer update was skipped, so weights, moments and step counters are unchanged.  NOT unchanged: the "
            "BatchNorm moving mean / variance, which the forward pass of the faulted step already advanced (a retried step "
            "applies that 1 % moving-average update a second time), and under data parallel the trip is per rank -- the other "
            "replicas have applied their update, so re-broadcast the parameters (dp.broadcast_parameters) before going on.  "
            "The model now uses the per-step LSTM kernels: run the step again.")

    def _guarded(self, fn):
# ... 409 lines not shown
```

### masters-thesis_amd/nic.py

```python
from collections import OrderedDict

import numpy as np
import torch

from .arena import ParamArena
from .model_base import (ModelBase, Metrics, _r4, S_IN, S_FEAT, S_LSTM_IN, BN_EPS, BN_MOMENTUM, S_SS_COIN, S_SS_DRAW,
                         SS_MAX_POSITIONS, S_SCST_LAST, ScheduledSampling, SelfCritical, check_sampling, check_beam,
                         _TokenChoice, _BeamDecode)
from .lstm_layer import lstm_layer_step_fwd, lstm_layer_fwd, lstm_layer_bwd
from .ops import ACT_LEAKY, LIVE_ROWS_M, LIVE_ROWS_K

ENC_SPLITS = 16


class NIC(ModelBase):
    BN = "batch_norm"

    def __init__(self, input_size, units, embedding_dim, vocab_size, max_length, dropout_input, dropout,
                 dropout_lstm, input_reg, lstm_reg, output_reg, norm="batch", scheduled_sampling=None, self_critical=None,
                 **kw):
        super().__init__(**kw)
        self.N, self.U, self.E, self.V, self.max_length = int(input_size), int(units), int(embedding_dim), int(vocab_size), int(max_length)
        self.r_in, self.r_feat, self.r_lstm = float(dropout_input), float(dropout), float(dropout_lstm)
        self.l2_in, self.l2_lstm, self.l2_out = float(input_reg), float(lstm_reg), float(lstm_reg)
# ... 1 lines not shown
        self.norm = norm
        if self.U % 16:
            raise ValueError("units must be a multiple of 16 (LSTM step kernel tile)")
        N, U, E, V = self.N, self.U, self.E, self.V
        if scheduled_sampling is not None:
            if not isinstance(scheduled_sampling, ScheduledSampling):
                raise ValueError("scheduled_sampling must be None or a model_base.ScheduledSampling, got "
                                 f"{scheduled_sampling!r}")
            if E % 4 or E > 1016:
                raise ValueError(f"scheduled sampling needs embedding_dim % 4 == 0 and <= 1016 "
                                 f"(tnt_scheduled_feedback_f32), got {E}")
        self.scheduled_sampling = scheduled_sampling
        if self_critical is not None:
            if not isinstance(self_critical, SelfCritical):
                raise ValueError(f"self_critical must be None or a model_base.SelfCritical, got {self_critical!r}")
            if scheduled_sampling is not None:
                raise ValueError("a model takes scheduled_sampling or self_critical, not both")
            if E % 4 or E > 1016:
                raise ValueError(f"self-critical training needs embedding_dim % 4 == 0 and <= 1016 "
                                 f"(tnt_scheduled_feedback_f32), got {E}")
            if self_critical.end_id >= V:
                raise ValueError(f"self-critical end_id {self_critical.end_id} is not below vocab_size {V}")
        self.self_critical = self_critical
        self._rollout_ss = ScheduledSampling.linear(1.0, 0.0, 1.0, mode="sample") if self_critical is not None else None
        self.ldx, self.ldV = _r4(N), _r4(V)
        self.layers_spec = OrderedDict([
            ("dense_img", ["kernel", "bias"]),
            ("batch_norm", ["gamma", "beta", "moving_mean", "moving_variance"]),
            ("emb_text", ["embeddings"]),
            ("lstm", ["kernel", "recurrent_kernel", "bias"]),
            ("time_distributed_softmax", ["kernel", "bias"])])
        self.keras_shapes = OrderedDict([
            ("dense_img/kernel", (N, E)), ("dense_img/bias", (E,)),
            ("batch_norm/gamma", (E,)), ("batch_norm/beta", (E,)),
            ("batch_norm/moving_mean", (E,)), ("batch_norm/moving_variance", (E,)),
            ("emb_text/embeddings", (V, E)),
            ("lstm/kernel", (E, 4 * U)), ("lstm/recurrent_kernel", (U, 4 * U)), ("lstm/bias", (4 * U,)),
            ("time_distributed_softmax/kernel", (U, V)), ("time_distributed_softmax/bias", (V,))])
        a = self.arena = ParamArena(self.device)
        a.add("dense_img/kernel", (N, E), self.l2_in)
        a.add("dense_img/bias", (E,))
        a.add("batch_norm/gamma", (E,))
        a.add("batch_norm/beta", (E,))
        a.add("emb_text/embeddings", (V, E))
        a.add("lstm/kernel", (E, U, 4), self.l2_lstm)
        a.add("lstm/recurrent_kernel", (U, U, 4))
        a.add("lstm/bias", (U, 4))
        a.add("time_distributed_softmax/kernel", (U, self.ldV), self.l2_out)
        a.add("time_distributed_softmax/bias", (self.ldV,))
        a.finalize()
        self.mov_mean, self.mov_var = self._f(E), torch.ones(E, dtype=torch.float32, device=self.device)
        self.drop_step = torch.zeros(1, dtype=torch.int32, device=self.device)
        if scheduled_sampling is not None or self_critical is not None:
            self.ss_sched = torch.tensor((scheduled_sampling or self._rollout_ss).params(), dtype=torch.float64,
                                         device=self.device)
        self._init_weights(np.random.default_rng(self.seed))
        self._shape = None

    def _init_weights(self, rng):
        N, U, E, V = self.N, self.U, self.E, self.V
        tn = lambda shape, std: np.clip(rng.standard_normal(shape), -2, 2) * std / 0.8796
        self.set_weight("dense_img/kernel", tn((N, E), np.sqrt(2.0 / (N + E))))
        self.set_weight("emb_text/embeddings", rng.uniform(-0.05, 0.05, (V, E)))
        lim = np.sqrt(6.0 / (E + 4 * U))
        self.set_weight("lstm/kernel", rng.uniform(-lim, lim, (E, 4 * U)))
        q = np.concatenate([np.linalg.qr(rng.standard_normal((U, U)))[0] for _ in range(4)], axis=1)
        self.set_weight("lstm/recurrent_kernel", q)
        b = np.zeros(4 * U); b[U:2 * U] = 1.0
        self.set_weight("lstm/bias", b)
        self.set_weight("time_distributed_softmax/kernel", tn((U, V), np.sqrt(2.0 / (U + V))))
        self.set_weight("batch_norm/gamma", np.ones(E))

    def _state_map(self):
        return {f"{self.BN}/moving_mean": self.mov_mean, f"{self.BN}/moving_variance": self.mov_var}

    def get_gradient(self, name):
        st = self.__dict__.get("_enc_grad_stale")
        if name == "dense_img/kernel" and st is not None:
            x, dpre, rows = st
            self.be.dense_dw_skinny(x, dpre, self.arena.g(name), self.N, self.E, rows, self.ldx)
            self._enc_grad_stale = None
        return super().get_gradient(name)

    def _enc_update_fused(self, rows):
        opt = self.optimizer
        return bool(self.__dict__.get("_defer_sum2") and self.dp_world == 1 and getattr(self, "fuse_enc_update", True)
                    and opt is not None and opt.kind == "adam" and not self.__dict__.get("agc") and rows <= 64
                    and self.E % 512 == 0 and hasattr(self.be, "dense_dw_adam") and hasattr(self.be, "step_finalize")
                    and self.arena.entries["dense_img/kernel"].seg == 0
                    and min((self.N + 15) // 16, 256) * (self.E // 512) <= self.arena.spans.first_host[1])

    def _build(self, B, T):
        if self._shape == (B, T):
            return
        f = self._f
        N, U, E, V, ldV = self.N, self.U, self.E, self.V, self.ldV
        R1 = (T + 1) * B
        self.x = f(B, self.ldx)
        self.xd = f(B, self.ldx) if self.r_in > 0 else self.x
        self.cap = torch.zeros(B, T, dtype=torch.int32, device=self.device)
        self.tgt = torch.zeros(T * B, dtype=torch.int32, device=self.device)
        self.enc_pre, self.enc_y = f(B, E), f(B, E)
        ok = self.norm == "batch" and B <= 256 and E % 32 == 0 and N % 4 == 0 and hasattr(self.be, "dense_fwd_stream")
        self.enc_part = f(ENC_SPLITS * B * E) if ok and getattr(self, "stream_encoder", True) else None
        self.enc_gx = self.enc_w2 = None
        self.enc_yd = f(B, E) if self.r_feat > 0 else self.enc_y
        self.xhat = f(B, E)
        self.inv_std = f(max(B, E))
        self.Xin = f(R1, E)
        self.Xin_d = f(R1, E) if self.r_lstm > 0 else self.Xin
        self.XZ = f(R1, U, 4)
        self.Hs, self.Cs = f(T + 2, B, U), f(T + 2, B, U)
        self.gates = f(T + 1, B, U, 4)
        self.Out = f(T, B, U)
        self._init_seq_lstm(B, U)
        self.logits = f(T * B, ldV)
        self.loss_row, self.corr_row = f(T * B), f(T * B)
        self.head_pos = torch.full((T * B,), -1, dtype=torch.int32, device=self.device)
        self.head_w = f(T * B)
        self.head_tgt = torch.zeros(T * B, dtype=torch.int32, device=self.device)
        self.head_live = torch.zeros(1, dtype=torch.int32, device=self.device)
        self._head_live_est = None
        self.met = f(8)
        self.dOut = f(T * B, U)
        self.dZ = f(R1, U, 4)
        self.da_pass, self.dc, self.dout = f(B, U), f(B, U), f(B, U)
        self.dXin = f(R1, E)
        self.dyd, self.dpre = f(B, E), f(B, E)
        be = self.be
        self._alloc_splitk([(B, E, N), (T * B, U, V), (R1, E, 4 * U), (R1, 4 * U, E), (T * B, V, U)])
        nch = max(be.bn_nchunk(B), be.bn_nchunk(R1), be.bn_nchunk(T * B))
        self.work = f(max(E, 4 * U, ldV) * (2 * nch + 1))
        self.work2 = f(max(E, 4 * U, ldV) * (2 * nch + 1))
        self.rowsq = f(B * T)
        self.emb_seg = self.arena.entries["emb_text/embeddings"].seg
        self._shape = (B, T)
        self._graphs = {}
        if self.optimizer is not None and getattr(self, "opt_m", None) is None:
            self._init_optimizer_state()
        self.built = True

    def _stage_inputs(self, data):
        x, cap, a0, c0 = data
        cap_t = self._to_dev(cap, torch.int32)
        B, T = cap_t.shape
        self._build(B, T)
        xs = self._to_dev(x, torch.float32)
        assert xs.shape == (B, self.N), f"betas shape {tuple(xs.shape)} != {(B, self.N)}"
        self.x[:, :self.N].copy_(xs)
        self.cap.copy_(cap_t)
        self.Hs[0].copy_(self._to_dev(a0, torch.float32))
        self.Cs[0].copy_(self._to_dev(c0, torch.float32))
        return B, T

    def _head_map_bufs(self, B, T):
        be = self.be
        ok = (getattr(self, "compact_head", True) and self.__dict__.get("_seq_lstm") and self.__dict__.get("seq_xch") is not None
              and hasattr(be, "stage_batch_map") and hasattr(be, "softmax_cce_live") and hasattr(be, "gemm3")
              and getattr(self, "use_gemm3", True) and getattr(self, "g3_riders", True)
              and self.grad_sync is None and int(self.__dict__.get("dp_world", 1) or 1) == 1
              and self.scheduled_sampling is None and self.self_critical is None and not self.__dict__.get("agc")
              and not self.label_smoothing and not self.unlikelihood and self.U % 4 == 0)
        if not ok:
            return None
        return (self.head_pos, self.head_w, self.head_tgt, self.head_live, self.loss_row, self.corr_row)

    def _fused_tail(self, B):
        return (self.norm == "batch" and B <= 256 and self.E % 4 == 0 and getattr(self, "fuse_tail", True)
                and not self._sync_bn_on())

    def _forward(self, B, T, training, ss=False):
        be, a = self.be, self.arena
        N, U, E, V, ldV = self.N, self.U, self.E, self.V, self.ldV
        R1 = (T + 1) * B
        sd, ds = self.seed, self.drop_step
        x = self.x
        if training and self.r_in > 0:
            be.dropout(self.x, self.xd, B, N, self.ldx, 0, N, 0, self.r_in, sd, S_IN, 0, ds)
            x = self.xd
        drop_l = training and self.r_lstm > 0
        xin = self.Xin_d if drop_l else self.Xin
        fused = self._fused_tail(B)
        stream = fused and self.enc_part is not None
        emb_ride = False
        if stream:
            self._enc_gram = None
            if (training and self._enc_update_fused(B) and getattr(self, "gram_norm", True) and N % 16 == 0 and E >= 512
                    and hasattr(be, "dense_gram_norm")):
                if self.enc_gx is None:
                    self.enc_gx, self.enc_w2 = self._f(ENC_SPLITS * 64 * 64), self._f(ENC_SPLITS * (E // 32))
                be.dense_fwd_stream_gram(x, a.p("dense_img/kernel"), self.enc_part, self.enc_gx, self.enc_w2, B, E, N,
                                         self.ldx, E, ENC_SPLITS)
                self._enc_gram = (self.enc_pre, a.p("dense_img/bias"), self.enc_gx, ENC_SPLITS, self.enc_w2,
                                  ENC_SPLITS * (E // 32))
            else:
                be.dense_fwd_stream(x, a.p("dense_img/kernel"), self.enc_part, B, E, N, self.ldx, E, ENC_SPLITS)
            emb_ride = E % 4 == 0 and hasattr(be, "enc_tail_fwd_sk_emb") and getattr(self, "emb_ride", True)
            targs = (self.enc_part, ENC_SPLITS, a.p("dense_img/bias"), self.enc_pre, 0.2, a.p("batch_norm/gamma"),
                     a.p("batch_norm/beta"), self.mov_mean, self.mov_var, xin, self.xhat, self.inv_std, B, E, E, training,
                     BN_EPS, BN_MOMENTUM, self.r_feat if training else 0.0, self.r_lstm if training else 0.0, sd, S_FEAT,
                     S_LSTM_IN + 0, ds)
            if emb_ride:
                be.enc_tail_fwd_sk_emb(*targs, a.p("emb_text/embeddings"), self.cap, xin[B:], B, T, V,
                                       self.r_lstm if drop_l else 0.0, S_LSTM_IN + 1)
            else:
                be.enc_tail_fwd_sk(*targs)
        else:
            self.gemm_sk(x, a.p("dense_img/kernel"), self.enc_y, B, E, N, self.ldx, E, E, bias=a.p("dense_img/bias"),
                         pre=self.enc_pre, act=ACT_LEAKY, slope=0.2)
        y = self.enc_y
        if stream:
            pass
        elif fused:
            be.enc_tail_fwd(y, a.p("batch_norm/gamma"), a.p("batch_norm/beta"), self.mov_mean, self.mov_var, xin,
                            self.xhat, self.inv_std, B, E, E, training, BN_EPS, BN_MOMENTUM,
                            self.r_feat if training else 0.0, self.r_lstm if training else 0.0, sd, S_FEAT,
                            S_LSTM_IN + 0, ds)
        else:
            if training and self.r_feat > 0:
                be.dropout(self.enc_y, self.enc_yd, B, E, E, 0, E, 0, self.r_feat, sd, S_FEAT, 0, ds)
                y = self.enc_yd
            if self.norm == "batch":
                self._bn_fwd(y, a.p("batch_norm/gamma"), a.p("batch_norm/beta"), self.mov_mean, self.mov_var,
                             self.Xin, self.xhat, self.inv_std, B, E, E, training, self.work)
            else:
                be.layernorm_fwd(y, a.p("batch_norm/gamma"), a.p("batch_norm/beta"), self.Xin, self.xhat,
                                 self.inv_std, B, E, E, BN_EPS)
        if drop_l and not fused:
            be.dropout(self.Xin, self.Xin_d, B, E, E, 0, E, 0, self.r_lstm, sd, S_LSTM_IN + 0, 0, ds)
        if stream and emb_ride:
            pass
        elif drop_l and E % 4 == 0:
            be.embedding_fwd_drop(a.p("emb_text/embeddings"), self.cap, None, self.Xin_d[B:], B, T, E, E, V, self.r_lstm,
                                  sd, S_LSTM_IN + 1, 0, ds)
        else:
            be.embedding_fwd(a.p("emb_text/embeddings"), self.cap, self.Xin[B:], B, T, E, E, V)
            if drop_l:
                be.dropout(self.Xin[B:], self.Xin_d[B:], T * B, E, E, B, E, 0, self.r_lstm, sd, S_LSTM_IN + 1, 0, ds)
        self._xin_used = xin
        if ss:
            self._forward_ss(B, T, xin, drop_l)
            return
        if getattr(self, "fused_xproj", False) and hasattr(be, "gemm_fused") and be.gemm_fused_cfg(R1, 4 * U, E) > 0:
            be.gemm_fused(xin, a.p("lstm/kernel"), self.XZ, R1, 4 * U, E, E, 4 * U, 4 * U)
        else:
            self.gemm_sk(xin, a.p("lstm/kernel"), self.XZ, R1, 4 * U, E, E, 4 * U, 4 * U)
        Ur, bl = a.p("lstm/recurrent_kernel"), a.p("lstm/bias")
        compact = bool(training and self.__dict__.get("_compact"))
        lstm_layer_fwd(be, self.XZ, self.Hs, self.Cs, Ur, bl, self.cap, T, 1, self.Out, self.gates, T + 1, B, U,
                       chain=self._seq_chain(), out_pos=self.head_pos if compact else None)
        if compact:
            self.gemm3(self.Out, a.p("time_distributed_softmax/kernel"), self.logits, T * B, V, U, U, ldV, ldV,
                       bias=a.p("time_distributed_softmax/bias"), live=self.head_live, live_mode=LIVE_ROWS_M,
                       plan_M=self._head_plan_rows(T * B))
            return
        self.gemm_sk(self.Out, a.p("time_distributed_softmax/kernel"), self.logits, T * B, V, U, U, ldV, ldV,
                bias=a.p("time_distributed_softmax/bias"))

    def _head_plan_rows(self, n):
        est = self._head_live_est
        if not getattr(self, "compact_head_replan", True) or est is None or est <= 0:
            return n
        return min(n, est + max(est // 32, 1))

    def _forward_ss(self, B, T, xin, drop_l):
        be, a = self.be, self.arena
        ss = self.scheduled_sampling if self.scheduled_sampling is not None else self._rollout_ss
        U, E, V, ldV = self.U, self.E, self.V, self.ldV
        Wl, Ur, bl = a.p("lstm/kernel"), a.p("lstm/recurrent_kernel"), a.p("lstm/bias")
        Wo, bo = a.p("time_distributed_softmax/kernel"), a.p("time_distributed_softmax/bias")
        table = a.p("emb_text/embeddings")
        self.gemm_sk(xin, Wl, self.XZ, 2 * B, 4 * U, E, E, 4 * U, 4 * U)
        step = lambda s: lstm_layer_step_fwd(be, s, self.XZ, self.Hs, self.Cs, Ur, bl, self.cap, T, 1, self.Out, self.gates,
                                             B, U)
        step(0)
        rate = self.r_lstm if drop_l else 0.0
        for t in range(1, T + 1):
# ... 150 lines not shown
        elif self.r_lstm > 0 and not fold:
            be.dropout(self.dXin[B:], self.dXin[B:], T * B, E, E, B, E, 0, self.r_lstm, sd, S_LSTM_IN + 1, 0, ds)
        self._emb_rows = (self.dXin[B:], T * B, E, E, "emb_text/embeddings")
        self._embedding_bwd(self.dXin[B:], self.cap, "emb_text/embeddings", B, T, E, E, V,
                            drop=(self.r_lstm, sd, S_LSTM_IN + 1, ds) if fold else None, zero_id=0)
        if ride:
            return
        if fused:
            be.enc_tail_bwd(self.dXin, self.xhat, a.p("batch_norm/gamma"), self.inv_std, self.enc_pre, self.dpre,
                            a.g("batch_norm/gamma"), a.g("batch_norm/beta"), a.g("dense_img/bias"), B, E, E,
                            self.r_feat, self.r_lstm, 0.2, sd, S_FEAT, S_LSTM_IN + 0, ds)
            return
        if self.norm == "batch":
            self._bn_bwd(self.dXin, self.xhat, a.p("batch_norm/gamma"), self.inv_std, self.dyd,
                         a.g("batch_norm/gamma"), a.g("batch_norm/beta"), B, E, E, self.work)
        else:
            be.layernorm_bwd(self.dXin, self.xhat, a.p("batch_norm/gamma"), self.inv_std, self.dyd,
                             a.g("batch_norm/gamma"), a.g("batch_norm/beta"), B, E, E, self.work)
        if self.r_feat > 0:
            be.dropout(self.dyd, self.dyd, B, E, E, 0, E, 0, self.r_feat, sd, S_FEAT, 0, ds)
        be.act_bwd(self.enc_pre, self.dyd, self.dpre, B * E, ACT_LEAKY, 0.2)
        be.colsum(self.dpre, a.g("dense_img/bias"), B, E, E, self.work)

    def _bwd_enc(self, B, T, x_all=None, dpre_all=None):
        be, a = self.be, self.arena
        x = self.xd if self.r_in > 0 else self.x
        rows = B
        if x_all is not None:
            x, dpre, rows = x_all, dpre_all, x_all.shape[0]
        else:
            dpre = self.dpre
        self._enc_last_fused = None
        if x_all is None and self._enc_update_fused(rows):
            self._enc_fused = ("dense_img/kernel", x, dpre, rows, self.N, self.E, self.ldx,
                               self.__dict__.get("_enc_gram"))
            self._enc_last_fused = (x, dpre, rows)
            return
        if rows <= 64 and self.E % 16 == 0 and getattr(self, "skinny_dw", True):
            be.dense_dw_skinny(x, dpre, a.g("dense_img/kernel"), self.N, self.E, rows, self.ldx)
        else:
            self.gemm_sk(x, dpre, a.g("dense_img/kernel"), self.N, self.E, rows, self.ldx, self.E, self.E, transA=True)

    def _enc_shard_state(self, r0, nr):
        st = self.__dict__.get("_enc_shard")
        if st is None or st["key"] != (r0, nr):
            from .arena import build_spans
            a, e = self.arena, self.arena.entries["dense_img/kernel"]
            assert e.seg == 0 and e.off == 0
            sp = build_spans([e.off + r0 * self.E], [nr * self.E], self.device)
            st = self._enc_shard = dict(key=(r0, nr), sp=sp, scratch=self._f(2 * sp.nspan), send=self._f(nr * self.E))
            a.partial[:2 * a.spans.first_host[1]].zero_()
        return st

    def _enc_shard_grad(self, x_all, dpre_all, r0, nr):
        be, a = self.be, self.arena
        st = self._enc_shard_state(r0, nr)
        sp = st["sp"]
        rows = x_all.shape[0]
        self.gemm_sk(x_all[:, r0:], dpre_all, a.g("dense_img/kernel")[r0:r0 + nr], nr, self.E, rows, self.ldx, self.E, self.E,
                     transA=True)
        be.seg_sqnorm(a.theta, a.grad, sp.span_seg, sp.span_off, sp.span_len, sp.seg_first, a.seg_l2, st["scratch"],
                      a.partial[0:1], a.partial[1:2], None, sp.nspan, 1)

    def _enc_shard_adam(self, r0, nr):
        be, a, opt = self.be, self.arena, self.optimizer
        st = self._enc_shard_state(r0, nr)
        sp = st["sp"]
        clip = opt.clipnorm if opt.clipnorm is not None else 0.0
        be.adam(a.theta, self.opt_m, self.opt_v, a.grad, sp.span_seg, sp.span_off, sp.span_len, a.seg_l2, a.partial[0:1],
                a.sq_override, sp.nspan, 0.0, self.lr_t_dev, opt.beta_1, opt.beta_2, opt.epsilon, clip, guard=self._guard_word())
        return st["send"]

    def _train_graph(self, B, T):
        self._forward(B, T, True, ss=self.scheduled_sampling is not None)
        self._loss_metrics(B, T, True)
        self._backward(B, T)

    def train_step(self, data):
        if self.optimizer is None:
            raise RuntimeError("compile() the model before train_step")
        self._ss_refuse()
        if self.self_critical is not None:
            return self.train_step_scst(data)
        B, T = self._stage_batch(data[0], data[1], self.N, head_map=self.grad_sync is None)
        self._ss_refuse(T)
        self._sync_lr()
        self._enc_grad_stale = None
        ring = False
        if self.grad_sync is None:
            compact = bool(self.__dict__.get("_head_map_fresh"))
            key = ("train", B, T, "compact") if compact else ("train", B, T)
            if compact and self._head_live_est is None and self._graphs.get(key) is None:
                self._head_live_est = int(self.head_live.item())
            self._compact = compact
            try:
                ring = self._run_step(self._step_runner(), key, lambda: self._train_and_update_graph(B, T))
            finally:
                self._compact = False
            self._enc_grad_stale = self.__dict__.get("_enc_last_fused")
        elif getattr(self.grad_sync, "pipelined", False):
            self.grad_sync.step(self, B, T)
        else:
            self._train_step_dp(B, T, lambda: self._train_graph(B, T), self._update_graph)
        self.optimizer.iterations += 1
        m = self._met_snapshot(ring)
        return self._metrics_from(m, loss=0, L2=2, accuracy=1)

    def _scst_bufs(self, B, T):
        R = B * self.self_critical.n_samples
        st = self.__dict__.get("_scst")
        if st is not None and st["key"] == (B, T):
            return st
        f, dev, i32 = self._f, self.device, torch.int32
        pin = self.device.type == "cuda"
        h = lambda *shape, dtype=i32: torch.zeros(*shape, dtype=dtype, pin_memory=pin)
        st = self._scst = dict(key=(B, T), x=f(B, self.ldx), h0=f(B, self.U), c0=f(B, self.U),
                               cap=torch.zeros(B, T, dtype=i32, device=dev), start=torch.zeros(B, 1, dtype=i32, device=dev),
                               greedy=torch.zeros(T, B, dtype=i32, device=dev), last=torch.zeros(R, dtype=i32, device=dev),
                               adv=f(R), h_cap=h(R, T), h_last=h(R), h_greedy=h(T, B), h_ref=h(B, T),
                               h_adv=h(R, dtype=torch.float32))
        return st

    def _stage_scst(self, inputs):
        x, cap, a0, c0 = inputs[:4]
        cap_t = self._to_dev(cap, torch.int32)
        B, T = cap_t.shape
        if T - 1 > SS_MAX_POSITIONS:
            raise ValueError(f"self-critical rollouts sample at most {SS_MAX_POSITIONS} token positions per caption through "
                             f"the scheduled-sampling sites (S_SS_DRAW + j): caption length {T} is too long")
        K = self.self_critical.n_samples
        self._build(B * K, T)
        st = self._scst_bufs(B, T)
        xs = self._to_dev(x, torch.float32)
        assert xs.shape == (B, self.N), f"betas shape {tuple(xs.shape)} != {(B, self.N)}"
        st["x"][:, :self.N].copy_(xs)
        st["h0"].copy_(self._to_dev(a0, torch.float32))
        st["c0"].copy_(self._to_dev(c0, torch.float32))
        st["cap"].copy_(cap_t)
        st["start"].copy_(cap_t[:, :1])
        self.x.view(B, K, self.ldx).copy_(st["x"][:, None, :].expand(B, K, self.ldx))
        self.Hs[0].view(B, K, self.U).copy_(st["h0"][:, None, :].expand(B, K, self.U))
        self.Cs[0].view(B, K, self.U).copy_(st["c0"][:, None, :].expand(B, K, self.U))
        self.cap.view(B, K, T).copy_(cap_t[:, None, :].expand(B, K, T))
        return B, T

    def _scst_greedy(self, B, T):
        be, a, st = self.be, self.arena, self._scst
        U, V, ldV = self.U, self.V, self.ldV
        h, c = [self.Hs[1][:B], self.Hs[2][:B]], [self.Cs[1][:B], self.Cs[2][:B]]
        self._decode_encode(B, (st["x"], st["h0"], st["c0"], h[0], c[0]))
        xz, emb, out, probs, ids = self.XZ[:B], self.Xin[B:2 * B], self.Out[0][:B], self.logits[:B], st["greedy"]
        for i in range(T):
            tok = st["start"] if i == 0 else ids[i - 1].view(B, 1)
            self._text_step(tok, i == 0, B, emb, xz, h[i & 1], c[i & 1], h[(i & 1) ^ 1], c[(i & 1) ^ 1], out,
                            self.gates[0][:B])
            self.gemm_sk(out, a.p("time_distributed_softmax/kernel"), probs, B, V, U, U, ldV, ldV,
                         bias=a.p("time_distributed_softmax/bias"))
            be.softmax_cce(probs, None, probs, None, None, None, B, V, ldV, 0.0)
            be.argmax_rows(probs, ids[i], B, V, ldV)

    def _scst_rollout(self, R, T):
        self._forward(R, T, True, ss=True)
        self.be.sample_rows(self.logits[(T - 1) * R:], self._scst["last"], R, self.V, self.ldV, 1.0, True, self.seed,
                            S_SCST_LAST, 0, self.drop_step)

    def _scst_update(self, R, T):
        st = self._scst
        self._defer_sum2 = True
        try:
            self.be.scst_cce(self.logits, self.ldV, self.V, self.cap, T, st["last"], st["adv"], self.self_critical.end_id,
                             self.loss_row, None, self.logits, R, 1.0 / R)
            self._sum2(self.loss_row, self.met[0:1], self.loss_row, self.met[1:2], T * R, 1.0 / R)
            self._backward(R, T)
        finally:
            self._defer_sum2 = False
        self._update_fused(self.met[2:3])

    def _scst_round_trip(self, B, T):
        st = self._scst
        pairs = [(st["h_cap"], self.cap), (st["h_last"], st["last"]), (st["h_ref"], st["cap"])]
        if self.self_critical.baseline == "greedy":
# ... 219 lines not shown
```

### masters-thesis_amd/ops.py

```python
import torch

from . import _lib

ACT_NONE, ACT_LEAKY, ACT_RELU, ACT_TANH = 0, 1, 2, 3


def _p(t):
    return None if t is None else t.data_ptr()


import ctypes as _ct


class _G3Desc(_ct.Structure):
    _fields_ = ([(n, _ct.c_void_p) for n in ("A", "B", "C", "bias", "colsum", "A2", "C2")]
                + [(n, _ct.c_int32) for n in ("M", "N", "K", "lda", "ldb", "ldc", "transA", "transB", "tile", "splitk")]
                + [(n, _ct.c_void_p) for n in ("work", "sync", "live")] + [("live_mode", _ct.c_int32)])


class _FinDesc(_ct.Structure):
    _fields_ = [("partial", _ct.c_void_p), ("seg_first", _ct.c_void_p), ("seg_l2", _ct.c_void_p), ("sq", _ct.c_void_p),
                ("wsq", _ct.c_void_p), ("l2_out", _ct.c_void_p), ("nseg", _ct.c_int32),
                ("x0", _ct.c_void_p), ("out0", _ct.c_void_p), ("x1", _ct.c_void_p), ("out1", _ct.c_void_p), ("n", _ct.c_int32),
                ("scale", _ct.c_float),
                ("extra_part", _ct.c_void_p), ("extra", _ct.c_void_p), ("n_extra", _ct.c_int32), ("extra_seg", _ct.c_int32),
                ("ids_src", _ct.c_void_p), ("ids_dst", _ct.c_void_p), ("n_ids", _ct.c_int32),
                ("x2", _ct.c_void_p), ("out2", _ct.c_void_p), ("n2", _ct.c_int32), ("scale2", _ct.c_float),
                ("adam_t", _ct.c_void_p), ("drop_step", _ct.c_void_p), ("lr", _ct.c_void_p), ("lr_t", _ct.c_void_p),
                ("beta1", _ct.c_float), ("beta2", _ct.c_float), ("guard", _ct.c_void_p), ("arrive", _ct.c_void_p)]


LIVE_ROWS_M, LIVE_ROWS_K = 1, 2


class HipBackend:
    name = "hip"

    def __init__(self):
        self.lib = _lib.load()
        if not torch.cuda.is_available():
            raise _lib.KernelLibraryError("no GPU visible: the HIP backend needs an MI355X (there is no CPU fallback)")

    _rec = None

    def _call(self, fn, name, *args):
        if self._rec is not None:
            self._rec.append((fn, name, args))
        rc = fn(*args)
        if rc != 0:
            raise _lib.KernelLibraryError(f"{name} failed with code {rc}")

    @staticmethod
    def _s():
        return torch._C._cuda_getCurrentRawStream(torch.cuda.current_device())

    def bn_nchunk(self, rows):
        return self.lib.tnt_bn_nchunk(rows)

    def gemm(self, A, B, C, M, N, K, lda, ldb, ldc, transA=False, transB=False, bias=None, pre=None,
             act=ACT_NONE, slope=0.2, accumulate=False, splitk=1, work=None):
        self._call(self.lib.tnt_gemm_f32, "tnt_gemm_f32", _p(A), _p(B), _p(C), _p(bias), _p(pre), M, N, K, lda, ldb, ldc,
                                         int(transA), int(transB), act, slope, int(accumulate), splitk,
                                         _p(work), self._s())

    def gemm_fused_cfg(self, M, N, K, transA=False, transB=False, batch=1):
        return int(self.lib.tnt_gemm_fused_cfg(M, N, K, int(transA), int(transB), batch))

    def gemm_fused(self, A, B, C, M, N, K, lda, ldb, ldc, transA=False, transB=False, bias=None, colsum=None, A2=None,
                   C2=None, cfg=0):
        self._call(self.lib.tnt_gemm_fused_f32, "tnt_gemm_fused_f32", _p(A), _p(B), _p(C), _p(bias), _p(colsum), _p(A2), _p(C2),
                   M, N, K, lda, ldb, ldc, int(transA), int(transB), cfg, self._s())

    def gemm3(self, A, B, C, M, N, K, lda, ldb, ldc, transA=False, transB=False, bias=None, colsum=None, A2=None, C2=None,
              tile=1, splitk=1, work=None, sync=None, live=None, live_mode=0):
        self._call(self.lib.tnt_gemm3_f32, "tnt_gemm3_f32", _p(A), _p(B), _p(C), _p(bias), _p(colsum), _p(A2), _p(C2),
                   M, N, K, lda, ldb, ldc, int(transA), int(transB), tile, splitk, _p(work), _p(sync), _p(live), int(live_mode),
                   self._s())

    def gemm3_plan(self, M, N, K, transA=False, transB=False, batch=1, allow_split=True):
        import ctypes
        t, s = ctypes.c_int32(0), ctypes.c_int32(1)
        rc = self.lib.tnt_gemm3_plan(M, N, K, int(transA), int(transB), batch, int(allow_split), ctypes.byref(t), ctypes.byref(s))
        if rc != 0:
            raise RuntimeError(f"tnt_gemm3_plan failed: {rc}")
        return int(t.value), int(s.value)

    def gemm3_work_floats(self, M, N, tile, splitk, batch=1):
        return int(self.lib.tnt_gemm3_work_floats(M, N, tile, splitk, batch))

    def gemm3_sync_words(self, M, N, tile, batch=1):
        return int(self.lib.tnt_gemm3_sync_words(M, N, tile, batch))

    def gemm3_pair(self, d1, d2):
        import ctypes
        self._call(self.lib.tnt_gemm3_pair_f32, "tnt_gemm3_pair_f32", ctypes.addressof(d1), ctypes.addressof(d2), self._s())

    def gemm3_pair_supported(self, tile1, tA1, tB1, tile2, tA2, tB2):
        return bool(self.lib.tnt_gemm3_pair_supported(tile1, int(tA1), int(tB1), tile2, int(tA2), int(tB2)))

    @staticmethod
    def gemm3_desc(A, B, C, M, N, K, lda, ldb, ldc, transA=False, transB=False, bias=None, colsum=None, A2=None, C2=None, tile=1,
                   splitk=1, work=None, sync=None, live=None, live_mode=0):
        d = _G3Desc(_p(A), _p(B), _p(C), _p(bias), _p(colsum), _p(A2), _p(C2), M, N, K, lda, ldb, ldc, int(transA), int(transB),
                    tile, splitk, _p(work), _p(sync), _p(live), int(live_mode))
        d._keep = (A, B, C, bias, colsum, A2, C2, work, sync, live)
        return d

    def gemm3_work_arm(self, work):
        self._call(self.lib.tnt_gemm3_work_arm, "tnt_gemm3_work_arm", _p(work), work.numel(), self._s())

    def gemm_tile(self, A, B, C, M, N, K, lda, ldb, ldc, bm, bn, transA=False, transB=False, bias=None, pre=None,
                  act=ACT_NONE, slope=0.2, accumulate=False, splitk=1, work=None):
        self._call(self.lib.tnt_gemm_f32_tile, "tnt_gemm_f32_tile", _p(A), _p(B), _p(C), _p(bias), _p(pre), M, N, K, lda, ldb, ldc,
                                              int(transA), int(transB), act, slope, int(accumulate), splitk,
                                              _p(work), bm, bn, self._s())

    def dropout(self, x, y, rows, cols, ld, tmajor_B, lwidth, lcol0, rate, seed, site, step, step_dev=None,
                rows_per_site=0):
        self._call(self.lib.tnt_dropout_f32, "tnt_dropout_f32", _p(x), _p(y), rows, cols, ld, tmajor_B, lwidth, lcol0, rows_per_site,
                                            rate, seed, site, step, _p(step_dev), self._s())

    def dropout_metric(self, x, y, rows, cols, ld, tmajor_B, lwidth, lcol0, rate, seed, site, step, step_dev, alpha, partial,
                       T, B, R, rows_per_site=0):
        self._call(self.lib.tnt_dropout_metric_f32, "tnt_dropout_metric_f32", _p(x), _p(y), rows, cols, ld, tmajor_B, lwidth,
                   lcol0, rows_per_site, rate, seed, site, step, _p(step_dev), _p(alpha), _p(partial), T, B, R, self._s())

    def dropout2(self, x, y, rows, cols, ld, mask_a, mask_b, seed, step, step_dev=None):
        self._call(self.lib.tnt_dropout2_f32, "tnt_dropout2_f32", _p(x), _p(y), rows, cols, ld, *[v for m in (mask_a, mask_b)
                   for v in (int(m[0]), int(m[1]), int(m[2]), int(m[3]), float(m[4]), int(m[5]))], int(seed), int(step),
                   _p(step_dev), self._s())

    def dropout_mask4(self, out, n, nsites, rate, seed, site0, step, step_dev=None):
        self._call(self.lib.tnt_dropout_mask4_u8, "tnt_dropout_mask4_u8", _p(out), n, nsites, rate, int(seed), int(site0), int(step), _p(step_dev),
# ... 118 lines not shown
                                                  _p(dout_in), _p(dout_t), _p(mask_ids), mask_T, mask_t, _p(gates),
                                                  _p(c), _p(c_prev), _p(dz), _p(da_pass_out), _p(dc_out),
                                                  _p(dout_out), B, U, _p(Wc), D, _p(dctx_part), self._s())

    def gru_step_fwd(self, xz, h_prev, Uk, br, h, gates, B, U):
        self._call(self.lib.tnt_gru_step_fwd_f32, "tnt_gru_step_fwd_f32", _p(xz), _p(h_prev), _p(Uk), _p(br), _p(h), _p(gates), B, U, self._s())

    def gru_step_bwd(self, drec_next, Uk, dh_pass_in, dh_ext, gates, h_prev, dxz, drec, dh_pass_out, B, U):
        self._call(self.lib.tnt_gru_step_bwd_f32, "tnt_gru_step_bwd_f32", _p(drec_next), _p(Uk), _p(dh_pass_in), _p(dh_ext), _p(gates), _p(h_prev),
                                                 _p(dxz), _p(drec), _p(dh_pass_out), B, U, self._s())

    def softmax_cce(self, logits, target, probs, loss_row, correct_row, dlogits, rows, V, ld, gscale,
                    from_logits=False, mask_zero=False):
        self._call(self.lib.tnt_softmax_cce_f32, "tnt_softmax_cce_f32", _p(logits), _p(target), _p(probs), _p(loss_row), _p(correct_row),
                                                _p(dlogits), rows, V, ld, gscale, int(from_logits), int(mask_zero),
                                                self._s())

    def softmax_cce_live(self, logits, target, probs, loss_row, correct_row, dlogits, rows, V, ld, gscale, live, row_weight):
        self._call(self.lib.tnt_softmax_cce_live_f32, "tnt_softmax_cce_live_f32", _p(logits), _p(target), _p(probs), _p(loss_row),
                   _p(correct_row), _p(dlogits), rows, V, ld, gscale, _p(live), _p(row_weight), self._s())

    def softmax_cce_smooth(self, logits, target, probs, loss_row, correct_row, dlogits, rows, V, ld, gscale, label_smoothing):
        self._call(self.lib.tnt_softmax_cce_smooth_f32, "tnt_softmax_cce_smooth_f32", _p(logits), _p(target), _p(probs), _p(loss_row),
                   _p(correct_row), _p(dlogits), rows, V, ld, gscale, float(label_smoothing), self._s())

    def softmax_cce_unlikely(self, logits, target, probs, loss_row, correct_row, dlogits, B, T, V, ld, gscale, alpha):
        self._call(self.lib.tnt_softmax_cce_unlikely_f32, "tnt_softmax_cce_unlikely_f32", _p(logits), _p(target), _p(probs),
                   _p(loss_row), _p(correct_row), _p(dlogits), B, T, V, ld, gscale, float(alpha), self._s())

    def onehot_argmax(self, onehot, ids_tmajor, B, T, V):
        self._call(self.lib.tnt_onehot_argmax_f32, "tnt_onehot_argmax_f32", _p(onehot), _p(ids_tmajor), B, T, V, self._s())

    def argmax_rows(self, x, out, rows, V, ld):
        self._call(self.lib.tnt_argmax_rows_f32, "tnt_argmax_rows_f32", _p(x), _p(out), rows, V, ld, self._s())

    def greedy_feedback(self, logits, ld, V, table, E, w, ldw, N, fed, T, col, text, ldt, xz, ldz, B, rate, seed, site, step,
                        step_dev=None, lwidth=0, lcol0=0):
        self._call(self.lib.tnt_greedy_feedback_f32, "tnt_greedy_feedback_f32", _p(logits), ld, V, _p(table), E, _p(w), ldw, N,
                   _p(fed), T, col, _p(text), ldt, _p(xz), ldz, B, float(rate), int(seed), int(site), int(step), _p(step_dev),
                   int(lwidth), int(lcol0), self._s())

    def scheduled_feedback(self, logits, ld, V, table, E, w, ldw, N, fed, T, col, text, ldt, xz, ldz, B, rate, seed, site,
                           step, step_dev, lwidth, lcol0, kind, mode, sched, counter, coin_site, draw_site):
        self._call(self.lib.tnt_scheduled_feedback_f32, "tnt_scheduled_feedback_f32", _p(logits), ld, V, _p(table), E, _p(w),
                   ldw, N, _p(fed), T, col, _p(text), ldt, _p(xz), ldz, B, float(rate), int(seed), int(site), int(step),
                   _p(step_dev), int(lwidth), int(lcol0), int(kind), int(mode), _p(sched), _p(counter),
                   int(coin_site), int(draw_site), self._s())

    def scheduled_feedback2(self, logits, ld, V, table, E, w, ldw, N, fed, T, col, text, ldt, xz, ldz, B, rate, seed, site,
                            step, step_dev, lwidth, lcol0, kind, mode, sched, counter, coin_site, draw_site, rate_t, site_t,
                            lwidth_t, lcol0_t):
        self._call(self.lib.tnt_scheduled_feedback2_f32, "tnt_scheduled_feedback2_f32", _p(logits), ld, V, _p(table), E,
                   _p(w), ldw, N, _p(fed), T, col, _p(text), ldt, _p(xz), ldz, B, float(rate), int(seed), int(site),
                   int(step), _p(step_dev), int(lwidth), int(lcol0), int(kind), int(mode), _p(sched), _p(counter),
                   int(coin_site), int(draw_site), float(rate_t), int(site_t), int(lwidth_t), int(lcol0_t), self._s())

    def enc_tail_fwd(self, y, gamma, beta, mov_mean, mov_var, out, xhat, inv_std, rows, C, ldo, training, eps, momentum,
                     r_feat, r_lstm, seed, site_feat, site_lstm, step_dev=None):
        self._call(self.lib.tnt_enc_tail_fwd_f32, "tnt_enc_tail_fwd_f32", _p(y), _p(gamma), _p(beta), _p(mov_mean), _p(mov_var), _p(out), _p(xhat),
                                                 _p(inv_std), rows, C, ldo, int(training), eps, momentum, r_feat, r_lstm,
                                                 int(seed), int(site_feat), int(site_lstm), _p(step_dev), self._s())

    def enc_tail_bwd_drop(self, dout, xhat, gamma, inv_std, pre, dpre, dgamma, dbeta, dbias, rows, C, ldo, r_feat, r_lstm,
                          slope, seed, site_feat, site_lstm, step_dev, drop_x, drop_rows, drop_cols, drop_ld, drop_tmajor_B,
                          drop_lwidth, drop_lcol0, drop_rate, drop_site):
        self._call(self.lib.tnt_enc_tail_bwd_drop_f32, "tnt_enc_tail_bwd_drop_f32", _p(dout), _p(xhat), _p(gamma), _p(inv_std),
                   _p(pre), _p(dpre), _p(dgamma), _p(dbeta), _p(dbias), rows, C, ldo, r_feat, r_lstm, slope, int(seed),
                   int(site_feat), int(site_lstm), _p(step_dev), _p(drop_x), drop_rows, drop_cols, drop_ld, drop_tmajor_B,
                   drop_lwidth, drop_lcol0, drop_rate, int(drop_site), self._s())

    def enc_tail_bwd(self, dout, xhat, gamma, inv_std, pre, dpre, dgamma, dbeta, dbias, rows, C, ldo, r_feat, r_lstm,
                     slope, seed, site_feat, site_lstm, step_dev=None):
        self._call(self.lib.tnt_enc_tail_bwd_f32, "tnt_enc_tail_bwd_f32", _p(dout), _p(xhat), _p(gamma), _p(inv_std), _p(pre), _p(dpre), _p(dgamma),
                                                 _p(dbeta), _p(dbias), rows, C, ldo, r_feat, r_lstm, slope, int(seed),
                                                 int(site_feat), int(site_lstm), _p(step_dev), self._s())

    def dense_fwd_stream(self, x, w, part, B, E, K, ldx, ldw, nsplit):
        self._call(self.lib.tnt_dense_fwd_stream_f32, "tnt_dense_fwd_stream_f32", _p(x), _p(w), _p(part), B, E, K, ldx, ldw,
                   nsplit, self._s())

    def dense_fwd_stream_gram(self, x, w, part, gx_part, w2_part, B, E, K, ldx, ldw, nsplit):
        self._call(self.lib.tnt_dense_fwd_stream_gram_f32, "tnt_dense_fwd_stream_gram_f32", _p(x), _p(w), _p(part), _p(gx_part),
                   _p(w2_part), B, E, K, ldx, ldw, nsplit, self._s())

    def dense_gram_norm(self, dpre, pre, bias, gx_part, nsplit, w2_part, nw2, l2, partial, nslot, Bk, E, spans=None, lr_job=None,
                        skip=None):
        if spans is not None and lr_job is not None:
            th, gr, sseg, soff, slen, sl2, spart, nspan = spans
            at, lr, lrt, b1, b2 = lr_job
            self._call(self.lib.tnt_dense_gram_norm_spans_lr_f32, "tnt_dense_gram_norm_spans_lr_f32", _p(dpre), _p(pre), _p(bias),
                       _p(gx_part), nsplit, _p(w2_part), nw2, l2, _p(partial), nslot, Bk, E, _p(th), _p(gr), _p(sseg), _p(soff),
                       _p(slen), _p(sl2), _p(spart), nspan, _p(at), _p(lr), _p(lrt), b1, b2, _p(skip), self._s())
            return
        if spans is None:
            self._call(self.lib.tnt_dense_gram_norm_f32, "tnt_dense_gram_norm_f32", _p(dpre), _p(pre), _p(bias), _p(gx_part), nsplit,
                       _p(w2_part), nw2, l2, _p(partial), nslot, Bk, E, self._s())
            return
        th, gr, sseg, soff, slen, sl2, spart, nspan = spans
        self._call(self.lib.tnt_dense_gram_norm_spans_f32, "tnt_dense_gram_norm_spans_f32", _p(dpre), _p(pre), _p(bias), _p(gx_part),
                   nsplit, _p(w2_part), nw2, l2, _p(partial), nslot, Bk, E, _p(th), _p(gr), _p(sseg), _p(soff), _p(slen), _p(sl2),
                   _p(spart), nspan, self._s())

    def enc_tail_fwd_sk_emb(self, part, nsplit, bias, pre, slope, gamma, beta, mov_mean, mov_var, out, xhat, inv_std, rows, C,
                            ldo, training, eps, momentum, r_feat, r_lstm, seed, site_feat, site_lstm, step_dev, emb_table,
                            emb_ids, emb_out, emb_B, emb_T, emb_V, emb_rate, emb_site):
        self._call(self.lib.tnt_enc_tail_fwd_sk_emb_f32, "tnt_enc_tail_fwd_sk_emb_f32", _p(part), nsplit, _p(bias), _p(pre), slope,
                   _p(gamma), _p(beta), _p(mov_mean), _p(mov_var), _p(out), _p(xhat), _p(inv_std), rows, C, ldo,
                   int(training), eps, momentum, r_feat, r_lstm, int(seed), int(site_feat), int(site_lstm), _p(step_dev),
                   _p(emb_table), _p(emb_ids), _p(emb_out), emb_B, emb_T, emb_V, emb_rate, int(emb_site), self._s())

    def enc_tail_fwd_sk(self, part, nsplit, bias, pre, slope, gamma, beta, mov_mean, mov_var, out, xhat, inv_std, rows, C,
                        ldo, training, eps, momentum, r_feat, r_lstm, seed, site_feat, site_lstm, step_dev=None):
        self._call(self.lib.tnt_enc_tail_fwd_sk_f32, "tnt_enc_tail_fwd_sk_f32", _p(part), nsplit, _p(bias), _p(pre), slope,
                   _p(gamma), _p(beta), _p(mov_mean), _p(mov_var), _p(out), _p(xhat), _p(inv_std), rows, C, ldo,
                   int(training), eps, momentum, r_feat, r_lstm, int(seed), int(site_feat), int(site_lstm), _p(step_dev),
                   self._s())

    def dense_dw_sqnorm(self, x, dpre, theta, l2, partial, nslot, N, E, Bk, ldx):
        self._call(self.lib.tnt_dense_dw_sqnorm_f32, "tnt_dense_dw_sqnorm_f32", _p(x), _p(dpre), _p(theta), l2, _p(partial),
                   nslot, N, E, Bk, ldx, self._s())

    def dense_dw_adam(self, x, dpre, theta, m, v, l2, sq, sq_override, lr_t_dev, beta1, beta2, eps, clipnorm, N, E, Bk, ldx,
                      guard=None):
        self._call(self.lib.tnt_dense_dw_adam_f32, "tnt_dense_dw_adam_f32", _p(x), _p(dpre), _p(theta), _p(m), _p(v), l2,
                   _p(sq), _p(sq_override), _p(lr_t_dev), beta1, beta2, eps, clipnorm, _p(guard), N, E, Bk, ldx, self._s())

    def dense_dw_skinny(self, x, dpre, dw, N, E, Bk, ldx):
        self._call(self.lib.tnt_dense_dw_skinny_f32, "tnt_dense_dw_skinny_f32", _p(x), _p(dpre), _p(dw), N, E, Bk, ldx, self._s())

    def lc_seq_fwd(self, F, P, W2, b2, v, bv, qpre, alpha, ctx, ctx_d, keep4, keep_stride, xz, Wc, Ur, xz_bias, hs, cs, gates, T,
                   B, R, D, A, U, slope, rate_attn, rate_in, in_lwidth, seed, site_attn0, site_in0, step_dev, work, sync,
                   guard_out=None, out_drop=None):
        if out_drop is not None:
            hd, rate_out, site_out0 = out_drop
            self._call(self.lib.tnt_lc_seq_fwd_drop_f32, "tnt_lc_seq_fwd_drop_f32", _p(F), _p(P), _p(W2), _p(b2), _p(v), _p(bv),
                       _p(qpre), _p(alpha), _p(ctx), _p(ctx_d), _p(keep4), int(keep_stride), _p(xz), _p(Wc), _p(Ur), _p(xz_bias),
                       _p(hs), _p(cs), _p(gates), T, B, R, D, A, U, slope, rate_attn, rate_in, in_lwidth, int(seed),
                       int(site_attn0), int(site_in0), _p(step_dev), _p(hd), float(rate_out), int(site_out0), _p(work), _p(sync),
                       _p(guard_out), self._s())
            return
        self._call(self.lib.tnt_lc_seq_fwd_f32, "tnt_lc_seq_fwd_f32", _p(F), _p(P), _p(W2), _p(b2), _p(v), _p(bv), _p(qpre), _p(alpha),
                   _p(ctx), _p(ctx_d), _p(keep4), int(keep_stride), _p(xz), _p(Wc), _p(Ur), _p(xz_bias), _p(hs), _p(cs), _p(gates),
                   T, B, R, D, A, U, slope, rate_attn, rate_in, in_lwidth, int(seed), int(site_attn0), int(site_in0),
                   _p(step_dev), _p(work), _p(sync), _p(guard_out), self._s())

    def lc_seq_fwd_work_floats(self, B):
        return int(self.lib.tnt_lc_seq_fwd_work_floats(int(B)))

    def lc_seq_bwd_work_floats(self, B, U):
        return int(self.lib.tnt_lc_seq_bwd_work_floats(int(B), int(U)))

    def lc_seq_bwd(self, F, P, W2, v, qpre, alpha, keep4, keep_stride, dP, dF, dvb, dqpre, Ur, Wc, dout, gates, cs, dz, work, T,
                   B, R, D, A, U, slope, rate_attn, rate_in, in_lwidth, seed, site_attn0, site_in0, step_dev, alpha_mse, sync,
                   guard_out=None, out_drop=None):
        if out_drop is not None:
            rate_out, site_out0 = out_drop
            self._call(self.lib.tnt_lc_seq_bwd_drop_f32, "tnt_lc_seq_bwd_drop_f32", _p(F), _p(P), _p(W2), _p(v), _p(qpre),
                       _p(alpha), _p(keep4), int(keep_stride), _p(dP), _p(dF), _p(dvb), _p(dqpre), _p(Ur), _p(Wc), _p(dout),
                       _p(gates), _p(cs), _p(dz), _p(work), T, B, R, D, A, U, slope, rate_attn, rate_in, in_lwidth, int(seed),
                       int(site_attn0), int(site_in0), _p(step_dev), float(alpha_mse), float(rate_out), int(site_out0),
                       _p(sync), _p(guard_out), self._s())
            return
        self._call(self.lib.tnt_lc_seq_bwd_f32, "tnt_lc_seq_bwd_f32", _p(F), _p(P), _p(W2), _p(v), _p(qpre), _p(alpha), _p(keep4),
                   int(keep_stride), _p(dP), _p(dF), _p(dvb), _p(dqpre), _p(Ur), _p(Wc), _p(dout), _p(gates), _p(cs), _p(dz),
                   _p(work), T, B, R, D, A, U, slope, rate_attn, rate_in, in_lwidth, int(seed), int(site_attn0), int(site_in0),
                   _p(step_dev), float(alpha_mse), _p(sync), _p(guard_out), self._s())
# ... 262 lines not shown
```

Before: 2.133 million caption-tokens/s.

## Fuse batch staging and row-map build into the encoder dense forward launch

Adds a staged variant of the Gram-form encoder dense forward kernel. It appends extra rider blocks to the grid that build the compacted head row map and copy the input batch, captions, targets and initial LSTM states. The goal is to run the separate stage_batch_map launch in parallel with the first dense GEMM instead of serializing it before the step. The encoder path then skips its own forward launch when staging already did it. Graph plans are invalidated when the staged mode changes, and a refusable call falls back to the old path.

```diff
diff --git a/include/tnt_hip.h b/include/tnt_hip.h
--- a/include/tnt_hip.h
+++ b/include/tnt_hip.h
@@ -152,6 +152,13 @@
 int32_t tnt_dense_fwd_stream_gram_f32(const float* x, const float* w, float* part, float* gx_part, float* w2_part,
                                       int32_t B, int32_t E, int32_t K, int32_t ldx, int32_t ldw, int32_t nsplit,
                                       void* stream);
+int32_t tnt_dense_fwd_stream_gram_stage_f32(const float* x, const float* w, float* part, float* gx_part, float* w2_part,
+                                            int32_t B, int32_t E, int32_t N, int32_t ldw, int32_t nsplit, float* x_dst,
+                                            int32_t ldx_dst, const int32_t* cap, int32_t* cap_dst, const int32_t* tgt,
+                                            int32_t* tgt_tmajor, const float* a0, float* h0, const float* c0,
+                                            float* c0_dst, int32_t T, int32_t U, int32_t* pos, float* row_weight,
+                                            int32_t* tgt_compact, int32_t* live, float* loss_row, float* corr_row,
+                                            void* stream);
 int32_t tnt_dense_gram_norm_f32(const float* dpre, const float* pre, const float* bias, const float* gx_part,
                                 int32_t nsplit, const float* w2_part, int32_t nw2, float l2, float* partial,
                                 int32_t nslot, int32_t Bk, int32_t E, void* stream);
diff --git a/masters-thesis_amd/_lib.py b/masters-thesis_amd/_lib.py
--- a/masters-thesis_amd/_lib.py
+++ b/masters-thesis_amd/_lib.py
@@ -87,6 +87,8 @@
     "tnt_dense_dw_sqnorm_f32": [P, P, P, F32, P, I32, I32, I32, I32, I32, P],
     "tnt_dense_dw_adam_f32": [P, P, P, P, P, F32, P, P, P, F32, F32, F32, F32, P, I32, I32, I32, I32, P],
     "tnt_dense_fwd_stream_gram_f32": [P, P, P, P, P, I32, I32, I32, I32, I32, I32, P],
+    "tnt_dense_fwd_stream_gram_stage_f32": [P, P, P, P, P, I32, I32, I32, I32, I32, P, I32, P, P, P, P, P, P, P, P, I32, I32,
+                                            P, P, P, P, P, P, P],
     "tnt_dense_gram_norm_f32": [P, P, P, P, I32, P, I32, F32, P, I32, I32, I32, P],
     "tnt_dense_gram_norm_spans_f32": [P, P, P, P, I32, P, I32, F32, P, I32, I32, I32, P, P, P, P, P, P, P, I32, P],
     "tnt_dense_fwd_stream_f32": [P, P, P, I32, I32, I32, I32, I32, I32, P],
diff --git a/masters-thesis_amd/csrc/encoder.hip b/masters-thesis_amd/csrc/encoder.hip
--- a/masters-thesis_amd/csrc/encoder.hip
+++ b/masters-thesis_amd/csrc/encoder.hip
@@ -1,5 +1,7 @@
 #include "tnt_common.h"
 #include "tnt_fin.h"
+#include "tnt_stage.h"
+#include <type_traits>
 
 namespace {
 
@@ -462,10 +464,21 @@
 constexpr int DF_CW = 32;
 
 struct DfArgs { const float* x; const float* w; float* part; int B, E, K, ldx, ldw, nsplit; float* gx_part; float* w2_part; };
-
-template <int NW, int DEPTH, bool GRAM>
-__global__ __launch_bounds__(64 * NW) void dense_fwd_stream_kernel(DfArgs a) {
+struct DfStageArgs : DfArgs { StageArgs<float> st; int nmain; };
+
+template <int NW, int DEPTH, bool GRAM, bool STAGE = false>
+__global__ __launch_bounds__(64 * NW) void dense_fwd_stream_kernel(std::conditional_t<STAGE, DfStageArgs, DfArgs> a) {
   __shared__ float red[NW][64][DF_CW + 4];
+  if constexpr (STAGE) {
+    static_assert(NW == 4, "the staging code expects 256 threads");
+    static_assert(sizeof(red) >= (3 * STAGE_MAP_LDS + 257) * sizeof(int), "the row map's LDS arrays live in red");
+    if ((int)blockIdx.x >= a.nmain) {
+      const int rider = blockIdx.x - a.nmain;
+      if (rider == 0) stage_rowmap_block(a.st, reinterpret_cast<int*>(&red[0][0][0]));
+      else stage_copy(a.st, rider - 1);
+      return;
+    }
+  }
   const int tid = threadIdx.x, lane = tid & 63, kq = lane >> 4, ln = lane & 15;
   const int w = __builtin_amdgcn_readfirstlane(tid >> 6);
   const int nct = a.E / DF_CW;
@@ -628,6 +641,44 @@
 extern "C" int32_t tnt_dense_fwd_stream_f32(const float* x, const float* w, float* part, int32_t B, int32_t E,
                                             int32_t K, int32_t ldx, int32_t ldw, int32_t nsplit, void* stream) {
   return dense_fwd_stream_launch(x, w, part, nullptr, nullptr, B, E, K, ldx, ldw, nsplit, stream);
+}
+
+extern "C" int32_t tnt_dense_fwd_stream_gram_stage_f32(const float* x, const float* w, float* part, float* gx_part,
+                                                       float* w2_part, int32_t B, int32_t E, int32_t N, int32_t ldw,
+                                                       int32_t nsplit, float* x_dst, int32_t ldx_dst, const int32_t* cap,
+                                                       int32_t* cap_dst, const int32_t* tgt, int32_t* tgt_tmajor,
+                                                       const float* a0, float* h0, const float* c0, float* c0_dst,
+                                                       int32_t T, int32_t U, int32_t* pos, float* row_weight,
+                                                       int32_t* tgt_compact, int32_t* live, float* loss_row,
+                                                       float* corr_row, void* stream) {
+  if (B <= 0 || B > 64 || N < 16 || N % 16 != 0) return TNT_BADARG(6);
+  if (E <= 0 || E % DF_CW != 0 || E / DF_CW < 16 || ldw < E || ldw % 2 != 0 || nsplit <= 0 || nsplit > 64) return TNT_BADARG(5);
+  if (gx_part == nullptr || w2_part == nullptr) return TNT_BADARG(4);
+  if (!tnt_aligned16(x) || !tnt_aligned16(w) || !tnt_aligned16(part)) return TNT_BADARG(1);
+  if ((long)B * N * 4 >= (1L << 32) || 16L * ldw * 4 >= (1L << 32)) return TNT_BADARG(4);
+  if (T <= 0 || U <= 0 || ldx_dst < N) return TNT_BADARG(11);
+  if (x_dst == nullptr || cap == nullptr || cap_dst == nullptr || a0 == nullptr || h0 == nullptr || c0 == nullptr ||
+      c0_dst == nullptr)
+    return TNT_BADARG(11);
+  if (pos == nullptr || row_weight == nullptr || tgt_compact == nullptr || live == nullptr || tgt == nullptr ||
+      tgt_tmajor == nullptr)
+    return TNT_BADARG(19);
+  if (ldx_dst % 4 == 0 && !tnt_aligned16(x_dst)) return TNT_BADARG(1);
+  DfStageArgs a{};
+  a.x = x; a.w = w; a.part = part; a.B = B; a.E = E; a.K = N; a.ldx = N; a.ldw = ldw; a.nsplit = nsplit;
+  a.gx_part = gx_part; a.w2_part = w2_part;
+  StageArgs<float>& s = a.st;
+  s.x = x; s.xd = x_dst; s.cap = cap; s.capd = cap_dst; s.tgt = tgt; s.tgtd = tgt_tmajor; s.a0 = a0; s.h0 = h0; s.c0 = c0;
+  s.c0d = c0_dst; s.B = B; s.T = T; s.N = N; s.ldx = ldx_dst; s.U = U;
+  s.map_pos = pos; s.map_w = row_weight; s.map_tgt = tgt_compact; s.map_live = live; s.map_loss = loss_row; s.map_corr = corr_row;
+  long nc = ((long)B * N / (ldx_dst % 4 == 0 ? 4 : 1) + 255) / 256;
+  s.ncopy = (int)(nc > 2048 ? 2048 : nc);
+  s.nstage = s.ncopy;
+  a.nmain = (E / DF_CW) * nsplit;
+  hipLaunchKernelGGL((dense_fwd_stream_kernel<4, 4, true, true>), dim3(a.nmain + 1 + s.ncopy), dim3(256), 0,
+                     tnt_stream(stream), a);
+  TNT_LAUNCH_CHECK();
+  return 0;
 }
 
 extern "C" int32_t tnt_dense_fwd_stream_gram_f32(const float* x, const float* w, float* part, float* gx_part,
diff --git a/masters-thesis_amd/csrc/rowops.hip b/masters-thesis_amd/csrc/rowops.hip
--- a/masters-thesis_amd/csrc/rowops.hip
+++ b/masters-thesis_amd/csrc/rowops.hip
@@ -1,6 +1,7 @@
 #include "tnt_common.h"
 #include <hip/hip_fp16.h>
 #include "tnt_rng.h"
+#include "tnt_stage.h"
 
 namespace {
 
@@ -356,138 +357,13 @@
   }
 }
 
-template <typename XT>
-struct StageArgs {
-  const XT* x; float* xd; const int* cap; int* capd; const int* tgt; int* tgtd;
-  const float* a0; float* h0; const float* c0; float* c0d;
-  int B, T, N, ldx, U;
-  float* xT; int ldt; int ncopy;
-  uint8_t* mk_out; long mk_n4, mk_total; float mk_rate; uint64_t mk_seed; uint32_t mk_site0; const uint32_t* mk_step_dev;
-  int nstage;
-  int* map_pos; float* map_w; int* map_tgt; int* map_live; float* map_loss; float* map_corr;
-};
-constexpr int STAGE_MAP_LDS = 1024;
-template <typename SA>
-__device__ __forceinline__ void stage_rowmap_lds(const SA& a, int* lds) {
-  int* s_cap = lds; int* s_tgt = lds + STAGE_MAP_LDS; int* s_pos = lds + 2 * STAGE_MAP_LDS; int* s_cnt = lds + 3 * STAGE_MAP_LDS;
-  const int B = a.B, T = a.T, n = B * T, tid = threadIdx.x;
-  for (int i = tid; i < n; i += 256) { s_cap[i] = a.cap[i]; s_tgt[i] = a.tgt[i]; }
-  __syncthreads();
-  for (int b = tid; b < B; b += 256) {
-    int rep_y = 0;
-    for (int t = 0; t < T; ++t) {
-      const int id = s_cap[b * T + t], y = s_tgt[b * T + t];
-      const bool merged = t > 0 && id == 0 && y == rep_y;
-      s_pos[t * B + b] = merged ? -1 : 1;
-      if (!merged) rep_y = y;
-    }
-  }
-  __syncthreads();
-  const int per = (n + 255) / 256, lo = min(tid * per, n), hi = min(lo + per, n);
-  int c = 0;
-  for (int i = lo; i < hi; ++i) c += s_pos[i] > 0 ? 1 : 0;
-  s_cnt[tid] = c;
-  __syncthreads();
-  if (tid == 0) {
-    int run = 0;
-    for (int k = 0; k < 256; ++k) { const int v = s_cnt[k]; s_cnt[k] = run; run += v; }
-    s_cnt[256] = run;
-    a.map_live[0] = run;
-  }
-  __syncthreads();
-  int idx = s_cnt[tid];
-  const int live = s_cnt[256];
-  for (int i = lo; i < hi; ++i)
-    if (s_pos[i] > 0) s_pos[i] = idx++;
-  __syncthreads();
-  for (int b = tid; b < B; b += 256) {
-    int rep = -1, cnt = 0;
-    for (int t = 0; t < T; ++t) {
-      const int p = s_pos[t * B + b];
-      if (p >= 0) {
-        if (rep >= 0) a.map_w[rep] = (float)cnt;
-        rep = p; cnt = 1;
-        a.map_tgt[p] = s_tgt[b * T + t];
-      } else {
-        ++cnt;
-      }
-    }
-    if (rep >= 0) a.map_w[rep] = (float)cnt;
-  }
-  for (int i = tid; i < n; i += 256) a.map_pos[i] = s_pos[i];
-  for (int i = live + tid; i < n; i += 256) {
-    a.map_w[i] = 0.f; a.map_tgt[i] = 0;
-    if (a.map_loss) a.map_loss[i] = 0.f;
-    if (a.map_corr) a.map_corr[i] = 0.f;
-  }
-}
-template <typename SA>
-__device__ __forceinline__ void stage_rowmap(const SA& a, int* s_cnt) {
-  const int B = a.B, T = a.T, n = B * T, tid = threadIdx.x;
-  for (int b = tid; b < B; b += 256) {
-    int rep_y = 0;
-    for (int t = 0; t < T; ++t) {
-      const int id = a.cap[b * T + t], y = a.tgt[b * T + t];
-      const bool merged = t > 0 && id == 0 && y == rep_y;
-      a.map_pos[t * B + b] = merged ? -1 : 1;
-      if (!merged) rep_y = y;
-    }
-  }
-  __syncthreads();
-  const int per = (n + 255) / 256, lo = min(tid * per, n), hi = min(lo + per, n);
-  int c = 0;
-  for (int i = lo; i < hi; ++i) c += a.map_pos[i] > 0 ? 1 : 0;
-  s_cnt[tid] = c;
-  __syncthreads();
-  if (tid == 0) {
-    int run = 0;
-    for (int k = 0; k < 256; ++k) { const int v = s_cnt[k]; s_cnt[k] = run; run += v; }
-    s_cnt[256] = run;
-    a.map_live[0] = run;
-  }
-  __syncthreads();
-  int idx = s_cnt[tid];
-  const int live = s_cnt[256];
-  for (int i = lo; i < hi; ++i)
-    if (a.map_pos[i] > 0) a.map_pos[i] = idx++;
-  __syncthreads();
-  for (int b = tid; b < B; b += 256) {
-    int rep = -1, cnt = 0;
-    for (int t = 0; t < T; ++t) {
-      const int p = a.map_pos[t * B + b];
-      if (p >= 0) {
-        if (rep >= 0) a.map_w[rep] = (float)cnt;
-        rep = p; cnt = 1;
-        a.map_tgt[p] = a.tgt[b * T + t];
-      } else {
-        ++cnt;
-      }
-    }
-    if (rep >= 0) a.map_w[rep] = (float)cnt;
-  }
-  for (int i = live + tid; i < n; i += 256) {
-    a.map_w[i] = 0.f; a.map_tgt[i] = 0;
-    if (a.map_loss) a.map_loss[i] = 0.f;
-    if (a.map_corr) a.map_corr[i] = 0.f;
-  }
-}
-__device__ __forceinline__ float stage_ld(const float* p) { return *p; }
-__device__ __forceinline__ float stage_ld(const __half* p) { return __half2float(*p); }
-__device__ __forceinline__ float4 stage_ld4(const float* p) { return *reinterpret_cast<const float4*>(p); }
-__device__ __forceinline__ float4 stage_ld4(const __half* p) {
-  const uint2 u = *reinterpret_cast<const uint2*>(p);
-  const __half2 lo = *reinterpret_cast<const __half2*>(&u.x), hi = *reinterpret_cast<const __half2*>(&u.y);
-  const float2 a = __half22float2(lo), b = __half22float2(hi);
-  return make_float4(a.x, a.y, b.x, b.y);
-}
 template <typename XT, bool MAP>
 __global__ __launch_bounds__(256) void stage_batch_kernel(StageArgs<XT> a) {
   __shared__ float tile[64][65];
   static_assert(sizeof(tile) >= (3 * STAGE_MAP_LDS + 257) * sizeof(int), "the row map's LDS arrays live in the tile");
   if (MAP && blockIdx.x == gridDim.x - 1) {
     int* lds = reinterpret_cast<int*>(&tile[0][0]);
-    if (a.B * a.T <= STAGE_MAP_LDS) stage_rowmap_lds(a, lds);
-    else stage_rowmap(a, lds);
+    stage_rowmap_block(a, lds);
     return;
   }
   if ((int)blockIdx.x >= a.nstage) {
@@ -518,25 +394,7 @@
     }
     return;
   }
-  const long gid = (long)blockIdx.x * 256 + threadIdx.x, gsz = (long)a.ncopy * 256;
-  if (a.N % 4 == 0 && a.ldx % 4 == 0) {
-    const int n4 = a.N / 4;
-    for (long e = gid; e < (long)a.B * n4; e += gsz) {
-      const int r = (int)(e / n4), c = (int)(e % n4) * 4;
-      *reinterpret_cast<float4*>(a.xd + (long)r * a.ldx + c) = stage_ld4(a.x + (long)r * a.N + c);
-    }
-  } else {
-    for (long e = gid; e < (long)a.B * a.N; e += gsz) {
-      const int r = (int)(e / a.N), c = (int)(e % a.N);
-      a.xd[(long)r * a.ldx + c] = stage_ld(a.x + e);
-    }
-  }
-  const int bt = a.B * a.T, bu = a.B * a.U;
-  for (long e = gid; e < bt; e += gsz) {
-    a.capd[e] = a.cap[e];
-    if (a.tgt) { const int b = (int)(e / a.T), t = (int)(e % a.T); a.tgtd[t * a.B + b] = a.tgt[e]; }
-  }
-  for (long e = gid; e < bu; e += gsz) { a.h0[e] = a.a0[e]; a.c0d[e] = a.c0[e]; }
+  stage_copy(a, blockIdx.x);
 }
 
 inline int ew_blocks(long total) {
@@ -1434,4 +1292,4 @@
                                     h0, c0, c0_dst, B, T, N, ldx, U, xT_dst, ldt, stream);
 }
 
-extern "C" int32_t tnt_version(void) { return 119; }
+extern "C" int32_t tnt_version(void) { return 120; }
diff --git a/masters-thesis_amd/csrc/tnt_stage.h b/masters-thesis_amd/csrc/tnt_stage.h
--- /dev/null
+++ b/masters-thesis_amd/csrc/tnt_stage.h
@@ -0,0 +1,159 @@
+#pragma once
+#include "tnt_common.h"
+#include <hip/hip_fp16.h>
+
+namespace {
+
+template <typename XT>
+struct StageArgs {
+  const XT* x; float* xd; const int* cap; int* capd; const int* tgt; int* tgtd;
+  const float* a0; float* h0; const float* c0; float* c0d;
+  int B, T, N, ldx, U;
+  float* xT; int ldt; int ncopy;
+  uint8_t* mk_out; long mk_n4, mk_total; float mk_rate; uint64_t mk_seed; uint32_t mk_site0; const uint32_t* mk_step_dev;
+  int nstage;
+  int* map_pos; float* map_w; int* map_tgt; int* map_live; float* map_loss; float* map_corr;
+};
+constexpr int STAGE_MAP_LDS = 1024;
+template <typename SA>
+__device__ __forceinline__ void stage_rowmap_lds(const SA& a, int* lds) {
+  int* s_cap = lds; int* s_tgt = lds + STAGE_MAP_LDS; int* s_pos = lds + 2 * STAGE_MAP_LDS; int* s_cnt = lds + 3 * STAGE_MAP_LDS;
+  const int B = a.B, T = a.T, n = B * T, tid = threadIdx.x;
+  for (int i = tid; i < n; i += 256) { s_cap[i] = a.cap[i]; s_tgt[i] = a.tgt[i]; }
+  __syncthreads();
+  for (int b = tid; b < B; b += 256) {
+    int rep_y = 0;
+    for (int t = 0; t < T; ++t) {
+      const int id = s_cap[b * T + t], y = s_tgt[b * T + t];
+      const bool merged = t > 0 && id == 0 && y == rep_y;
+      s_pos[t * B + b] = merged ? -1 : 1;
+      if (!merged) rep_y = y;
+    }
+  }
+  __syncthreads();
+  const int per = (n + 255) / 256, lo = min(tid * per, n), hi = min(lo + per, n);
+  int c = 0;
+  for (int i = lo; i < hi; ++i) c += s_pos[i] > 0 ? 1 : 0;
+  s_cnt[tid] = c;
+  __syncthreads();
+  if (tid == 0) {
+    int run = 0;
+    for (int k = 0; k < 256; ++k) { const int v = s_cnt[k]; s_cnt[k] = run; run += v; }
+    s_cnt[256] = run;
+    a.map_live[0] = run;
+  }
+  __syncthreads();
+  int idx = s_cnt[tid];
+  const int live = s_cnt[256];
+  for (int i = lo; i < hi; ++i)
+    if (s_pos[i] > 0) s_pos[i] = idx++;
+  __syncthreads();
+  for (int b = tid; b < B; b += 256) {
+    int rep = -1, cnt = 0;
+    for (int t = 0; t < T; ++t) {
+      const int p = s_pos[t * B + b];
+      if (p >= 0) {
+        if (rep >= 0) a.map_w[rep] = (float)cnt;
+        rep = p; cnt = 1;
+        a.map_tgt[p] = s_tgt[b * T + t];
+      } else {
+        ++cnt;
+      }
+    }
+    if (rep >= 0) a.map_w[rep] = (float)cnt;
+  }
+  for (int i = tid; i < n; i += 256) a.map_pos[i] = s_pos[i];
+  for (int i = live + tid; i < n; i += 256) {
+    a.map_w[i] = 0.f; a.map_tgt[i] = 0;
+    if (a.map_loss) a.map_loss[i] = 0.f;
+    if (a.map_corr) a.map_corr[i] = 0.f;
+  }
+}
+template <typename SA>
+__device__ __forceinline__ void stage_rowmap(const SA& a, int* s_cnt) {
+  const int B = a.B, T = a.T, n = B * T, tid = threadIdx.x;
+  for (int b = tid; b < B; b += 256) {
+    int rep_y = 0;
+    for (int t = 0; t < T; ++t) {
+      const int id = a.cap[b * T + t], y = a.tgt[b * T + t];
+      const bool merged = t > 0 && id == 0 && y == rep_y;
+      a.map_pos[t * B + b] = merged ? -1 : 1;
+      if (!merged) rep_y = y;
+    }
+  }
+  __syncthreads();
+  const int per = (n + 255) / 256, lo = min(tid * per, n), hi = min(lo + per, n);
+  int c = 0;
+  for (int i = lo; i < hi; ++i) c += a.map_pos[i] > 0 ? 1 : 0;
+  s_cnt[tid] = c;
+  __syncthreads();
+  if (tid == 0) {
+    int run = 0;
+    for (int k = 0; k < 256; ++k) { const int v = s_cnt[k]; s_cnt[k] = run; run += v; }
+    s_cnt[256] = run;
+    a.map_live[0] = run;
+  }
+  __syncthreads();
+  int idx = s_cnt[tid];
+  const int live = s_cnt[256];
+  for (int i = lo; i < hi; ++i)
+    if (a.map_pos[i] > 0) a.map_pos[i] = idx++;
+  __syncthreads();
+  for (int b = tid; b < B; b += 256) {
+    int rep = -1, cnt = 0;
+    for (int t = 0; t < T; ++t) {
+      const int p = a.map_pos[t * B + b];
+      if (p >= 0) {
+        if (rep >= 0) a.map_w[rep] = (float)cnt;
+        rep = p; cnt = 1;
+        a.map_tgt[p] = a.tgt[b * T + t];
+      } else {
+        ++cnt;
+      }
+    }
+    if (rep >= 0) a.map_w[rep] = (float)cnt;
+  }
+  for (int i = live + tid; i < n; i += 256) {
+    a.map_w[i] = 0.f; a.map_tgt[i] = 0;
+    if (a.map_loss) a.map_loss[i] = 0.f;
+    if (a.map_corr) a.map_corr[i] = 0.f;
+  }
+}
+__device__ __forceinline__ float stage_ld(const float* p) { return *p; }
+__device__ __forceinline__ float stage_ld(const __half* p) { return __half2float(*p); }
+__device__ __forceinline__ float4 stage_ld4(const float* p) { return *reinterpret_cast<const float4*>(p); }
+__device__ __forceinline__ float4 stage_ld4(const __half* p) {
+  const uint2 u = *reinterpret_cast<const uint2*>(p);
+  const __half2 lo = *reinterpret_cast<const __half2*>(&u.x), hi = *reinterpret_cast<const __half2*>(&u.y);
+  const float2 a = __half22float2(lo), b = __half22float2(hi);
+  return make_float4(a.x, a.y, b.x, b.y);
+}
+template <typename SA>
+__device__ __forceinline__ void stage_rowmap_block(const SA& a, int* lds) {
+  if (a.B * a.T <= STAGE_MAP_LDS) stage_rowmap_lds(a, lds);
+  else stage_rowmap(a, lds);
+}
+template <typename SA>
+__device__ __forceinline__ void stage_copy(const SA& a, int blk) {
+  const long gid = (long)blk * 256 + threadIdx.x, gsz = (long)a.ncopy * 256;
+  if (a.N % 4 == 0 && a.ldx % 4 == 0) {
+    const int n4 = a.N / 4;
+    for (long e = gid; e < (long)a.B * n4; e += gsz) {
+      const int r = (int)(e / n4), c = (int)(e % n4) * 4;
+      *reinterpret_cast<float4*>(a.xd + (long)r * a.ldx + c) = stage_ld4(a.x + (long)r * a.N + c);
+    }
+  } else {
+    for (long e = gid; e < (long)a.B * a.N; e += gsz) {
+      const int r = (int)(e / a.N), c = (int)(e % a.N);
+      a.xd[(long)r * a.ldx + c] = stage_ld(a.x + e);
+    }
+  }
+  const int bt = a.B * a.T, bu = a.B * a.U;
+  for (long e = gid; e < bt; e += gsz) {
+    a.capd[e] = a.cap[e];
+    if (a.tgt) { const int b = (int)(e / a.T), t = (int)(e % a.T); a.tgtd[t * a.B + b] = a.tgt[e]; }
+  }
+  for (long e = gid; e < bu; e += gsz) { a.h0[e] = a.a0[e]; a.c0d[e] = a.c0[e]; }
+}
+
+}
diff --git a/masters-thesis_amd/model_base.py b/masters-thesis_amd/model_base.py
--- a/masters-thesis_amd/model_base.py
+++ b/masters-thesis_amd/model_base.py
@@ -1257,7 +1257,10 @@
     def _head_map_bufs(self, B, T):
         return None
 
-    def _stage_batch(self, inputs, target, n_cols, masks=False, head_map=False):
+    def _stage_fwd_args(self, B):
+        return None
+
+    def _stage_batch(self, inputs, target, n_cols, masks=False, head_map=False, fwd=False):
         x, cap, a0, c0 = inputs[:4]
         if target is not None and self.unlikelihood > 0 and np.shape(cap)[-1] > self.UNLIKELIHOOD_MAX_T:
             raise ValueError(f"unlikelihood training holds a caption's prefix in one wave: at most {self.UNLIKELIHOOD_MAX_T} "
@@ -1271,6 +1274,7 @@
         ok = ok and x.dim() == 2 and cap.dim() == 2 and x.shape == (cap.shape[0], n_cols)
         ok = ok and (target is None or (target.dtype == torch.int32 and target.shape == cap.shape))
         self._head_map_fresh = False
+        self._stage_fwd_done = False
         if not ok:
             B, T = self._stage_inputs(inputs)
             if target is not None:
@@ -1289,7 +1293,12 @@
             kw["masks"] = mk
         hm = self._head_map_bufs(B, T) if (head_map and target is not None and mk is None and xT is None
                                            and x.dtype == torch.float32) else None
-        if hm is not None:
+        sf = self._stage_fwd_args(B) if (fwd and hm is not None and n_cols == self.ldx) else None
+        if sf is not None and self.be.dense_fwd_stream_gram_stage(x, *sf[:4], B, sf[4], n_cols, sf[5], sf[6], self.x, self.ldx,
+                                                                  cap, self.cap, target, self.tgt, a0, self.Hs[0], c0,
+                                                                  self.Cs[0], T, self.U, *hm):
+            self._head_map_fresh = self._stage_fwd_done = True
+        elif hm is not None:
             self.be.stage_batch_map(x, self.x, cap, self.cap, target, self.tgt, a0, self.Hs[0], c0, self.Cs[0], B, T, n_cols,
                                     self.ldx, self.U, *hm)
             self._head_map_fresh = True
diff --git a/masters-thesis_amd/nic.py b/masters-thesis_amd/nic.py
--- a/masters-thesis_amd/nic.py
+++ b/masters-thesis_amd/nic.py
@@ -107,9 +107,10 @@
             self._enc_grad_stale = None
         return super().get_gradient(name)
 
-    def _enc_update_fused(self, rows):
+    def _enc_update_fused(self, rows, defer=None):
         opt = self.optimizer
-        return bool(self.__dict__.get("_defer_sum2") and self.dp_world == 1 and getattr(self, "fuse_enc_update", True)
+        defer = self.__dict__.get("_defer_sum2") if defer is None else defer
+        return bool(defer and self.dp_world == 1 and getattr(self, "fuse_enc_update", True)
                     and opt is not None and opt.kind == "adam" and not self.__dict__.get("agc") and rows <= 64
                     and self.E % 512 == 0 and hasattr(self.be, "dense_dw_adam") and hasattr(self.be, "step_finalize")
                     and self.arena.entries["dense_img/kernel"].seg == 0
@@ -190,6 +191,23 @@
             return None
         return (self.head_pos, self.head_w, self.head_tgt, self.head_live, self.loss_row, self.corr_row)
 
+    def _gram_fwd(self, B, defer=None):
+        return (self._fused_tail(B) and self.enc_part is not None and self._enc_update_fused(B, defer)
+                and getattr(self, "gram_norm", True) and self.N % 16 == 0 and self.E >= 512
+                and hasattr(self.be, "dense_gram_norm"))
+
+    def _gram_bufs(self):
+        if self.enc_gx is None:
+            self.enc_gx, self.enc_w2 = self._f(ENC_SPLITS * 64 * 64), self._f(ENC_SPLITS * (self.E // 32))
+
+    def _stage_fwd_args(self, B):
+        ok = (getattr(self, "stage_fwd", True) and self.r_in == 0 and hasattr(self.be, "dense_fwd_stream_gram_stage")
+              and self._gram_fwd(B, defer=bool(getattr(self, "fused_update", True))))
+        if not ok:
+            return None
+        self._gram_bufs()
+        return (self.arena.p("dense_img/kernel"), self.enc_part, self.enc_gx, self.enc_w2, self.E, self.E, ENC_SPLITS)
+
     def _fused_tail(self, B):
         return (self.norm == "batch" and B <= 256 and self.E % 4 == 0 and getattr(self, "fuse_tail", True)
                 and not self._sync_bn_on())
@@ -210,14 +228,16 @@
         emb_ride = False
         if stream:
             self._enc_gram = None
-            if (training and self._enc_update_fused(B) and getattr(self, "gram_norm", True) and N % 16 == 0 and E >= 512
-                    and hasattr(be, "dense_gram_norm")):
-                if self.enc_gx is None:
-                    self.enc_gx, self.enc_w2 = self._f(ENC_SPLITS * 64 * 64), self._f(ENC_SPLITS * (E // 32))
-                be.dense_fwd_stream_gram(x, a.p("dense_img/kernel"), self.enc_part, self.enc_gx, self.enc_w2, B, E, N,
-                                         self.ldx, E, ENC_SPLITS)
+            staged = bool(training and self.__dict__.get("_stage_fwd"))
+            if training and self._gram_fwd(B):
+                self._gram_bufs()
+                if not staged:
+                    be.dense_fwd_stream_gram(x, a.p("dense_img/kernel"), self.enc_part, self.enc_gx, self.enc_w2, B, E, N,
+                                             self.ldx, E, ENC_SPLITS)
                 self._enc_gram = (self.enc_pre, a.p("dense_img/bias"), self.enc_gx, ENC_SPLITS, self.enc_w2,
                                   ENC_SPLITS * (E // 32))
+            elif staged:
+                raise RuntimeError("the staging launch ran the Gram form of the encoder forward, which this step does not take")
             else:
                 be.dense_fwd_stream(x, a.p("dense_img/kernel"), self.enc_part, B, E, N, self.ldx, E, ENC_SPLITS)
             emb_ride = E % 4 == 0 and hasattr(be, "enc_tail_fwd_sk_emb") and getattr(self, "emb_ride", True)
@@ -534,21 +554,26 @@
         self._ss_refuse()
         if self.self_critical is not None:
             return self.train_step_scst(data)
-        B, T = self._stage_batch(data[0], data[1], self.N, head_map=self.grad_sync is None)
+        B, T = self._stage_batch(data[0], data[1], self.N, head_map=self.grad_sync is None, fwd=self.grad_sync is None)
         self._ss_refuse(T)
         self._sync_lr()
         self._enc_grad_stale = None
         ring = False
         if self.grad_sync is None:
             compact = bool(self.__dict__.get("_head_map_fresh"))
+            staged = bool(self.__dict__.get("_stage_fwd_done"))
             key = ("train", B, T, "compact") if compact else ("train", B, T)
+            seen = self.__dict__.setdefault("_plan_staged", {})
+            if self._graphs.get(key) is not None and seen.get(key) != staged:
+                del self._graphs[key]
+            seen[key] = staged
             if compact and self._head_live_est is None and self._graphs.get(key) is None:
                 self._head_live_est = int(self.head_live.item())
-            self._compact = compact
+            self._compact, self._stage_fwd = compact, staged
             try:
                 ring = self._run_step(self._step_runner(), key, lambda: self._train_and_update_graph(B, T))
             finally:
-                self._compact = False
+                self._compact = self._stage_fwd = False
             self._enc_grad_stale = self.__dict__.get("_enc_last_fused")
         elif getattr(self.grad_sync, "pipelined", False):
             self.grad_sync.step(self, B, T)
diff --git a/masters-thesis_amd/ops.py b/masters-thesis_amd/ops.py
--- a/masters-thesis_amd/ops.py
+++ b/masters-thesis_amd/ops.py
@@ -43,12 +43,20 @@
 
     _rec = None
 
-    def _call(self, fn, name, *args):
-        if self._rec is not None:
-            self._rec.append((fn, name, args))
-        rc = fn(*args)
+    def _call(self, fn, name, *args, may_refuse=False):
+        if may_refuse:
+            rc = fn(*args)
+            if rc <= -1000:
+                return False
+            if self._rec is not None:
+                self._rec.append((fn, name, args))
+        else:
+            if self._rec is not None:
+                self._rec.append((fn, name, args))
+            rc = fn(*args)
         if rc != 0:
             raise _lib.KernelLibraryError(f"{name} failed with code {rc}")
+        return True
 
     @staticmethod
     def _s():
@@ -333,6 +341,14 @@
     def dense_fwd_stream_gram(self, x, w, part, gx_part, w2_part, B, E, K, ldx, ldw, nsplit):
         self._call(self.lib.tnt_dense_fwd_stream_gram_f32, "tnt_dense_fwd_stream_gram_f32", _p(x), _p(w), _p(part), _p(gx_part),
                    _p(w2_part), B, E, K, ldx, ldw, nsplit, self._s())
+
+    def dense_fwd_stream_gram_stage(self, x, w, part, gx_part, w2_part, B, E, N, ldw, nsplit, x_dst, ldx_dst, cap, cap_dst, tgt,
+                                    tgt_tmajor, a0, h0, c0, c0_dst, T, U, pos, row_weight, tgt_compact, live, loss_row=None,
+                                    corr_row=None):
+        return self._call(self.lib.tnt_dense_fwd_stream_gram_stage_f32, "tnt_dense_fwd_stream_gram_stage_f32", _p(x), _p(w),
+                          _p(part), _p(gx_part), _p(w2_part), B, E, N, ldw, nsplit, _p(x_dst), ldx_dst, _p(cap), _p(cap_dst),
+                          _p(tgt), _p(tgt_tmajor), _p(a0), _p(h0), _p(c0), _p(c0_dst), T, U, _p(pos), _p(row_weight),
+                          _p(tgt_compact), _p(live), _p(loss_row), _p(corr_row), self._s(), may_refuse=True)
 
     def dense_gram_norm(self, dpre, pre, bias, gx_part, nsplit, w2_part, nw2, l2, partial, nslot, Bk, E, spans=None, lr_job=None,
                         skip=None):
```

Result: faster. 2.175 million caption-tokens/s, median of 6 (+2.0%).
